# nayuki/DEFLATE-library-Java

Measured on AMD Instinct MI355X. Metric: input MiB/s (compress+decompress), higher is better.
Workload: dtype u8

## Files before the change

deflate-library-java_amd/csrc/hip/inflate_kernels.hip:

```cpp
#pragma once
#include "ndfl_common.hpp"
#include "../../../include/ndfl.h"
#include <vector>
#include <algorithm>
#include <unordered_map>
#include <chrono>
#include <string.h>
#include <stdio.h>
#include <stdlib.h>

namespace inf {

constexpr uint32_t SEG_BYTES = 65536;
constexpr uint32_t SEG_CAP = 256;
constexpr uint64_t NONE = ~0ull;

enum : uint32_t { ST_BOUNDARY = 0, ST_FINAL = 1, ST_ERROR = 2 };
constexpr int NEED_INPUT = 64;
enum : int { R_UEOS = 1, R_RESERVED_BLOCK_TYPE, R_LEN_MISMATCH, R_UNDER_FULL, R_OVER_FULL, R_NO_PREV,
             R_CL_OVER_FULL, R_EOB_ZERO, R_RESERVED_LEN, R_RESERVED_DIST, R_EMPTY_DIST, R_COPY_BEFORE,
             R_RESERVED_LEN_HI = 20, R_RESERVED_DIST_HI = 21,
             R_INTERNAL = 100 };

constexpr int CLO[19] = {16, 17, 18, 0, 8, 7, 9, 6, 10, 5, 11, 4, 12, 3, 13, 2, 14, 1, 15};
// ... 422 lines not shown
    __device__ __forceinline__ uint32_t pick8(uint32_t i) const {
        const uint32_t a = pick(cur, i), b = pick(nxt, i);
        return (i & 4) ? b : a;
    }
    __device__ __forceinline__ void load(const In& in, uint64_t g) {
        qw = g;
        cur = in.ld4(g);
        nxt = in.ld4(g + 1);
    }
    __device__ __forceinline__ uint64_t bits64(uint32_t o) const {
        const uint32_t i = o >> 5, sh = o & 31;
        const uint64_t x = (uint64_t)pick8(i) | ((uint64_t)pick8(i + 1) << 32);
        return sh ? (x >> sh) | ((uint64_t)pick8(i + 2) << (64 - sh)) : x;
    }
    __device__ __forceinline__ void fill() {
        if (bn <= 32 && fi < 8) { bb |= (uint64_t)pick8(fi) << bn; bn += 32; fi++; }
    }
    __device__ __forceinline__ void seek(uint64_t p) {
        pos = p;
        const uint32_t o = (uint32_t)(p - qw * 128);
        fi = o >> 5;
        bb = (uint64_t)(pick8(fi) >> (o & 31));
        bn = 32 - (o & 31);
        fi++;
        fill();
    }
    __device__ __forceinline__ bool starved() const { return bn <= 32 && fi >= 8; }
    __device__ __forceinline__ void reload(const In& in) {
        const uint64_t wn = qw * 4 + fi;
        load(in, wn >> 2);
        fi = (uint32_t)wn & 3u;
    }
    __device__ __forceinline__ uint32_t peek(uint32_t n) const { return (uint32_t)bb & ((1u << n) - 1u); }
    __device__ __forceinline__ void skip(uint32_t n) { bb >>= n; bn -= n; pos += n; }
};
}

extern "C" __global__ void __launch_bounds__(256) __attribute__((amdgpu_waves_per_eu(NDFL_STRICT_WPE)))
ndfl_inflate_strict_kernel(const uint32_t* w, uint64_t nwords, uint64_t nbits, const uint64_t* qlist,
                           const uint32_t* qcount, uint32_t qcap, uint32_t* seg_cnt, uint64_t* seg_list,
                           uint32_t* ticket, unsigned long long* sst) {
    using namespace inf;
    __shared__ uint4 tabs[256 * 8];
    uint8_t* tab = (uint8_t*)&tabs[threadIdx.x * 8];
    const uint32_t n = min(*qcount, qcap);
    In in{w, nwords, nbits};
    const uint32_t lane = threadIdx.x & 63u;
    uint32_t next = 0, end = 0;
    bool drained = false;
    const uint64_t below = (1ull << lane) - 1ull;
    auto record = [&](uint64_t p) {
        const uint32_t seg = (uint32_t)(p / ((uint64_t)SEG_BYTES * 8));
        const uint32_t idx = atomicAdd(&seg_cnt[seg], 1u);
        if (idx < SEG_CAP) seg_list[(uint64_t)seg * SEG_CAP + idx] = p;
    };
    bool active = false;
    uint64_t p = 0;
    SRd rd;
    rd.bb = 0; rd.pos = 0; rd.qw = 0; rd.bn = 0; rd.fi = 8;
    uint32_t i = 0, total = 0, numLit = 0, numDist = 0, litK = 0, distK = 0, nz = 0, eob = 0;
    int runVal = -1;
    uint64_t n_iter = 0, n_refill = 0, n_steps = 0;
    for (;;) {
        const uint64_t idle = __ballot(!active);
        const uint32_t nidle = (uint32_t)__popcll(idle);
        n_iter++;
        if (next >= end && !drained && nidle >= NDFL_STRICT_REFILL) {
            uint32_t t = 0;
            if (lane == 0) t = atomicAdd(ticket, STRICT_SLICE);
            t = __shfl(t, 0);
            if (t >= n) drained = true;
            else { next = t; end = min(n, t + STRICT_SLICE); }
        }
        if (next < end && nidle >= NDFL_STRICT_REFILL) {
            n_refill++;
            if (!active) {
                const uint32_t k = next + (uint32_t)__popcll(idle & below);
                if (k < end) {
                    const uint64_t e = qlist[k];
                    p = e & ~(1ull << 63);
                    if (!(e >> 63)) {
                        if (strict_stored(in, p)) record(p);
                    } else {
                        rd.load(in, p >> 7);
                        const uint32_t o = (uint32_t)p & 127u;
                        const uint32_t h = (uint32_t)rd.bits64(o + 3);
                        const uint32_t hlit = h & 31u, hdist = (h >> 5) & 31u, hclen = (h >> 10) & 15u;
                        numLit = hlit + 257; numDist = hdist + 1; total = numLit + numDist;
                        const uint32_t numCl = hclen + 4;
                        const uint64_t F = rd.bits64(o + 17) & ((1ull << (3 * numCl)) - 1ull);
                        rd.seek(p + 17 + 3 * numCl);
                        uint64_t wp = 0;
                        uint32_t kraft = 0;
#pragma unroll
                        for (int sy = 0; sy < 19; sy++) {
                            const uint32_t l = (uint32_t)(F >> (3 * CLO_INV[sy])) & 7u;
                            wp += l ? ((uint64_t)(128u >> l) << (8 * l)) : 0ull;
                            kraft += l ? (128u >> l) : 0u;
                        }
                        const bool complete = kraft == 128u;
                        uint64_t off = (wp * 0x0101010101010101ull) << 8;
#pragma unroll 1
                        for (int sy = 0; sy < 19; sy++) {
                            const uint32_t l = (uint32_t)(F >> (3 * CLO_INV[sy])) & 7u;
                            if (l && complete) {
                                const uint32_t sh = 8 * l, run = 128u >> l;
                                const uint32_t pos = (uint32_t)(off >> sh) & 255u;
                                off += (uint64_t)run << sh;
                                const uint32_t v = ((uint32_t)sy | (l << 5)) * 0x01010101u;
                                if (run >= 16) {
                                    for (uint32_t r = 0; r < run; r += 16) *(uint4*)(tab + pos + r) = make_uint4(v, v, v, v);
                                } else if (run == 8) {
                                    *(uint2*)(tab + pos) = make_uint2(v, v);
                                } else if (run == 4) {
                                    *(uint32_t*)(tab + pos) = v;
                                } else if (run == 2) {
                                    *(uint16_t*)(tab + pos) = (uint16_t)v;
                                } else {
                                    tab[pos] = (uint8_t)v;
                                }
                            }
                        }
                        i = 0; runVal = -1; litK = 0; distK = 0; nz = 0; eob = 0;
                        active = complete;
                    }
                }
            }
            next = min(end, next + nidle);
            continue;
        }
        if (!__any(active)) {
            if (next >= end && drained) break;
            continue;
        }
        const bool more = next < end || !drained;
        for (uint32_t ni = nidle;;) {
        n_steps += 64 - ni;
        if (__any(active && rd.starved())) {
            if (active && rd.fi >= 4) rd.reload(in);
        }
        if (active) {
            rd.fill();
            const uint32_t b = (uint32_t)rd.bb;
            const uint32_t te = tab[__builtin_bitreverse32(b) >> 25];
            const uint32_t sym = te & 31u, cl = te >> 5;
            const bool s16 = sym == 16, s17 = sym == 17, s18 = sym == 18;
            const uint32_t nx = s16 ? 2u : s17 ? 3u : s18 ? 7u : 0u;
            const uint32_t ex = (b >> cl) & ((1u << nx) - 1u);
            const uint32_t run = sym < 16 ? 1u : ex + (s18 ? 11u : 3u);
            const bool bad = s16 && runVal < 0;
            runVal = sym < 16 ? (int)sym : s16 ? runVal : 0;
            rd.skip(cl + nx);
            const uint32_t en = i + run;
            const uint32_t v = (uint32_t)runVal;
            const uint32_t wt = v ? (32768u >> v) : 0u;
            litK += (min(en, numLit) - min(i, numLit)) * wt;
            const uint32_t da = max(i, numLit) - numLit, db = max(en, numLit) - numLit, cd = db - da;
            distK += cd * wt;
            nz += v ? cd : 0u;
            eob = (i <= 256 && 256 < en) ? v : eob;
            i = en;
            const bool go = !(bad || en > total) && litK <= 32768u && distK <= 32768u;
            active = go && i < total;
            if (go && i >= total) {
                bool ok;
                if (eob == 0 || litK != 32768u || rd.pos > in.nbits) ok = false;
                else if (numDist == 1 && distK == 0) ok = true;
                else if (nz == 1 && distK == 16384u) ok = true;
                else ok = distK == 32768u;
                if (ok) record(p);
            }
        }
        const uint64_t am = __ballot(active);
        ni = 64u - (uint32_t)__popcll(am);
        if (!am || (more && ni >= NDFL_STRICT_REFILL)) break;
        n_iter++;
        }
    }
    if (sst && lane == 0) {
        atomicAdd(&sst[0], (unsigned long long)n_iter);
        atomicAdd(&sst[1], (unsigned long long)n_refill);
        atomicAdd(&sst[2], (unsigned long long)n_steps);
        atomicAdd(&sst[3], 1ull);
    }
}
extern "C" __global__ void __launch_bounds__(256)
ndfl_inflate_compact_kernel(const uint32_t* seg_cnt, const uint64_t* seg_list, const uint64_t* seg_off,
                            uint32_t nseg, uint64_t* out) {
    using namespace inf;
    __shared__ uint64_t sv[4][SEG_CAP];
    const uint32_t wid = threadIdx.x >> 6, lane = threadIdx.x & 63u;
    const uint32_t seg = blockIdx.x * 4 + wid;
    if (seg >= nseg) return;
    const uint32_t c = min(seg_cnt[seg], SEG_CAP);
    const uint64_t* src = seg_list + (uint64_t)seg * SEG_CAP;
    uint64_t* o = out + seg_off[seg];
    static_assert(SEG_CAP == 256, "four candidates per lane");
    uint64_t v[4];
#pragma unroll
    for (int q = 0; q < 4; q++) {
        const uint32_t i = lane + 64u * q;
        v[q] = i < c ? src[i] : ~0ull;
        if (i < c) sv[wid][i] = v[q];
    }
    __builtin_amdgcn_fence(__ATOMIC_RELEASE, "wavefront");
    __builtin_amdgcn_wave_barrier();
    __builtin_amdgcn_fence(__ATOMIC_ACQUIRE, "wavefront");
    uint32_t r[4] = {0, 0, 0, 0};
    for (uint32_t j = 0; j < c; j++) {
        const uint64_t u = sv[wid][j];
#pragma unroll
        for (int q = 0; q < 4; q++) r[q] += u < v[q] ? 1u : 0u;
    }
#pragma unroll
    for (int q = 0; q < 4; q++)
        if (lane + 64u * q < c) o[r[q]] = v[q];
}

struct ChainRes {
    uint64_t end_bit;
    uint64_t out_count;
    uint32_t status;
    uint32_t reason;
    uint32_t next;
    uint32_t pad;
    uint64_t bnd_bit;
    uint64_t bnd_cnt;
};

struct EmitChain {
    uint64_t start_bit;
    uint64_t end_bit;
    uint64_t out_off;
    uint64_t out_count;
    uint64_t slot;
};

enum : uint32_t { LI_NCAND = 0, LI_NCH, LI_TOTAL, LI_FLAGS, LI_STOP, LI_CODE, LI_OUTLEN, LI_CONSUMED, LI_NCAND_ALL,
                  LI_LO, LI_NREP, LI_NFLAT, LI_WORDS = 16 };
enum : uint64_t { LF_REPAIR = 1, LF_RANGE = 2, LF_CAPACITY = 4 };
constexpr uint32_t NOLINK = 0xFFFFFFFFu;

extern "C" __global__ void __launch_bounds__(SCAN_T)
ndfl_inflate_segsum_kernel(const uint32_t* cnt, uint32_t nseg, uint64_t* part) {
    using namespace inf;
    scan_tile_sum([&](uint32_t i) { return (uint64_t)min(cnt[i], SEG_CAP); }, nseg, part);
}
extern "C" __global__ void __launch_bounds__(SCAN_T)
ndfl_inflate_segscan_kernel(const uint32_t* cnt, uint32_t nseg, uint64_t* segoff, uint64_t* info, const uint64_t* part) {
    using namespace inf;
    scan_tile_apply([&](uint32_t i) { return (uint64_t)min(cnt[i], SEG_CAP); },
                    [&](uint32_t i, uint64_t v) { segoff[i] = v; }, nseg, part, 1, info + LI_NCAND_ALL);
}

extern "C" __global__ void __launch_bounds__(256)
ndfl_inflate_cand_slice_kernel(const uint64_t* sorted, uint64_t* info, uint64_t start_bit, uint64_t end_bit,
                               uint64_t* cands) {
    __shared__ uint64_t s_lo, s_hi;
    const uint64_t na = info[LI_NCAND_ALL];
    if (threadIdx.x == 0) {
        uint64_t lo = 1, hi = na;
        while (lo < hi) { const uint64_t m = (lo + hi) >> 1; if (sorted[m] <= start_bit) lo = m + 1; else hi = m; }
        uint64_t lo2 = lo, hi2 = na;
        while (lo2 < hi2) { const uint64_t m = (lo2 + hi2) >> 1; if (sorted[m] < end_bit) lo2 = m + 1; else hi2 = m; }
        s_lo = lo; s_hi = lo2;
        if (blockIdx.x == 0) { info[LI_NCAND] = 1 + (lo2 - lo); info[LI_LO] = lo; cands[0] = start_bit; }
    }
    __syncthreads();
    const uint64_t lo = s_lo, n = s_hi - s_lo;
    for (uint64_t k = (uint64_t)blockIdx.x * 256 + threadIdx.x; k < n; k += (uint64_t)gridDim.x * 256)
        cands[1 + k] = sorted[lo + k];
}

__device__ __forceinline__ uint64_t stored_key(const inf::In& in, uint64_t p) {
    const uint32_t h = (uint32_t)in.win64(p) & 7u;
    if ((h >> 1) != 0 || p + 3 > in.nbits) return ~0ull;
    return (((p + 3 + 7) & ~7ull) << 1) | (h & 1u);
}

extern "C" __global__ void __launch_bounds__(256)
ndfl_inflate_alias_mark_kernel(const uint64_t* cands, uint64_t* info, const uint32_t* w, uint64_t nwords, uint64_t nbits,
                               uint32_t* rep) {
    const inf::In in{w, nwords, nbits};
    const uint32_t n = (uint32_t)min<uint64_t>(info[LI_NCAND], 0xFFFFFFFFull);
    for (uint32_t k0 = blockIdx.x * 256; k0 < n; k0 += gridDim.x * 256) {
        const uint32_t k = k0 + threadIdx.x;
        bool own = false;
        if (k < n) {
            const uint64_t p = cands[k], key = stored_key(in, p);
            uint32_t r = k;
            if (key != ~0ull)
                for (uint32_t j = k; j > 0 && cands[j - 1] + 10 >= p; j--)
                    if (stored_key(in, cands[j - 1]) == key) r = j - 1;
            rep[k] = r;
            own = r == k;
        }
        const uint32_t c = (uint32_t)__popcll(__ballot(own));
        if ((threadIdx.x & 63) == 0 && c) atomicAdd((unsigned long long*)&info[LI_NREP], (unsigned long long)c);
    }
}

constexpr uint32_t OB_NB = 24;
constexpr uint32_t OB_WORDS = 2 * OB_NB;
constexpr size_t CTK_BYTES = 512;

template <class Bk>
__device__ __forceinline__ void border_count(Bk bk, uint32_t n, uint32_t* ob) {
    __shared__ uint32_t h[OB_NB];
    const uint32_t t = threadIdx.x;
    if (t < OB_NB) h[t] = 0;
    __syncthreads();
    const uint32_t i0 = blockIdx.x * SCAN_TILE + t * SCAN_PER;
    if (i0 < n) {
        uint32_t b[SCAN_PER];
#pragma unroll
        for (uint32_t k = 0; k < SCAN_PER; k++) b[k] = bk(min(i0 + k, n - 1));
#pragma unroll
        for (uint32_t k = 0; k < SCAN_PER; k++) if (i0 + k < n && b[k] < OB_NB) atomicAdd(&h[b[k]], 1u);
    }
    __syncthreads();
    if (t < OB_NB && h[t]) atomicAdd(&ob[t], h[t]);
}
template <class Bk>
__device__ __forceinline__ void border_place(Bk bk, uint32_t n, uint32_t* ob, uint32_t* order, uint32_t* ntot) {
    __shared__ uint32_t h[OB_NB], base[OB_NB];
    const uint32_t t = threadIdx.x;
    if (t < OB_NB) h[t] = 0;
    __syncthreads();
    const uint32_t i0 = blockIdx.x * SCAN_TILE + t * SCAN_PER;
    uint32_t b[SCAN_PER];
#pragma unroll
    for (uint32_t k = 0; k < SCAN_PER; k++) b[k] = OB_NB;
    if (i0 < n) {
#pragma unroll
        for (uint32_t k = 0; k < SCAN_PER; k++) b[k] = bk(min(i0 + k, n - 1));
#pragma unroll
        for (uint32_t k = 0; k < SCAN_PER; k++) {
            if (i0 + k >= n) b[k] = OB_NB;
            if (b[k] < OB_NB) atomicAdd(&h[b[k]], 1u);
        }
    }
    __syncthreads();
    if (t < OB_NB) {
        uint32_t p = 0;
        for (uint32_t q = 0; q < t; q++) p += ob[q];
        base[t] = p + (h[t] ? atomicAdd(&ob[OB_NB + t], h[t]) : 0u);
        h[t] = 0;
    }
    __syncthreads();
#pragma unroll
    for (uint32_t k = 0; k < SCAN_PER; k++)
        if (b[k] < OB_NB) order[base[b[k]] + atomicAdd(&h[b[k]], 1u)] = i0 + k;
    if (ntot && blockIdx.x == 0 && t == 0) {
        uint32_t p = 0;
        for (uint32_t q = 0; q < OB_NB; q++) p += ob[q];
        *ntot = p;
    }
}

struct OrderBucket {
    const uint64_t* cands; uint32_t n; uint64_t end_bit; const uint32_t* rep; const uint32_t* flat;
    __device__ __forceinline__ uint32_t operator()(uint32_t k) const {
        const uint64_t c0 = cands[k], c1 = cands[min(k + 1, n - 1)];
        const uint32_t r = rep ? rep[k] : k;
        const uint64_t nx = k + 1 < n ? c1 : end_bit;
        const uint64_t len = nx > c0 ? nx - c0 : 0;
        if (flat && flat[k]) return OB_NB;
        return r == k ? OB_NB - 1 - (uint32_t)min<uint64_t>(OB_NB - 1, len >> 15) : OB_NB;
    }
};
extern "C" __global__ void __launch_bounds__(SCAN_T)
ndfl_inflate_order_count_kernel(const uint64_t* cands, uint32_t n, uint64_t end_bit, const uint32_t* rep, uint32_t* ob,
                                const uint32_t* flat) {
    border_count(OrderBucket{cands, n, end_bit, rep, flat}, n, ob);
}
extern "C" __global__ void __launch_bounds__(SCAN_T)
ndfl_inflate_order_kernel(const uint64_t* cands, uint32_t n, uint64_t end_bit, uint32_t* order, const uint32_t* rep,
                          uint32_t* nord, uint32_t* ob, const uint32_t* flat) {
    border_place(OrderBucket{cands, n, end_bit, rep, flat}, n, ob, order, nord);
}

struct EmitBucket {
    const EmitChain* chains;
    __device__ __forceinline__ uint32_t operator()(uint32_t k) const {
        const EmitChain& e = chains[k];
        const uint64_t key = ((e.end_bit - e.start_bit) >> 15) + (e.out_count >> 14);
        return OB_NB - 1 - (uint32_t)min<uint64_t>(OB_NB - 1, key);
    }
};
extern "C" __global__ void __launch_bounds__(SCAN_T)
ndfl_inflate_emit_order_count_kernel(const EmitChain* chains, const uint64_t* info, uint32_t* ob) {
    if (info[LI_FLAGS]) return;
    border_count(EmitBucket{chains}, (uint32_t)info[LI_NCH], ob);
}
extern "C" __global__ void __launch_bounds__(SCAN_T)
ndfl_inflate_emit_order_kernel(const EmitChain* chains, const uint64_t* info, uint32_t* order, uint32_t* ob) {
    if (info[LI_FLAGS]) return;
    border_place(EmitBucket{chains}, (uint32_t)info[LI_NCH], ob, order, (uint32_t*)nullptr);
}

extern "C" __global__ void __launch_bounds__(256)
ndfl_inflate_link_init_kernel(const ChainRes* res, uint32_t n, const uint64_t* cands, uint64_t end_bit, uint32_t* J0,
                              uint64_t* S, uint32_t* D) {
    using namespace inf;
    for (uint32_t k = blockIdx.x * 256 + threadIdx.x; k < n; k += gridDim.x * 256) {
        const ChainRes r = res[k];
        const bool lk = r.status == ST_BOUNDARY && r.end_bit < end_bit && r.next < n && cands[r.next] == r.end_bit;
        J0[k] = lk ? r.next : NOLINK;
        S[k] = r.out_count;
        D[k] = lk ? 1u : 0u;
    }
}
extern "C" __global__ void __launch_bounds__(256)
ndfl_inflate_link_jump_kernel(const uint32_t* J, uint32_t* J2, const uint64_t* S, uint64_t* S2, const uint32_t* D,
                              uint32_t* D2, uint32_t n) {
    for (uint32_t k = blockIdx.x * 256 + threadIdx.x; k < n; k += gridDim.x * 256) {
        const uint32_t j = J[k];
        if (j != NOLINK) { J2[k] = J[j]; S2[k] = S[k] + S[j]; D2[k] = D[k] + D[j]; }
        else { J2[k] = NOLINK; S2[k] = S[k]; D2[k] = D[k]; }
    }
}
extern "C" __global__ void __launch_bounds__(256)
ndfl_inflate_link_path_kernel(const uint32_t* Jall, uint32_t nlev, const uint64_t* S, const uint32_t* D,
                              const ChainRes* res, const uint64_t* cands, uint32_t n, uint64_t dict_len, uint64_t end_bit,
                              uint64_t out_cap, EmitChain* chains, uint64_t* info) {
    using namespace inf;
    const uint32_t len = D[0] + 1;
    for (uint32_t t = blockIdx.x * 256 + threadIdx.x; t < len; t += gridDim.x * 256) {
        uint32_t node = 0;
        for (uint32_t r = 0; r < nlev; r++)
            if ((t >> r) & 1u) node = Jall[(uint64_t)r * n + node];
        const ChainRes c = res[node];
        EmitChain e;
        e.start_bit = cands[node];
        e.end_bit = c.end_bit;
        e.out_off = dict_len + S[0] - S[node];
        e.out_count = c.out_count;
        e.slot = node;
        chains[t] = e;
        if (t + 1 == len) {
            uint64_t flags = 0, stop = 0;
            if (c.status == ST_FINAL) stop = c.end_bit;
            else if (c.status == ST_BOUNDARY) {
                if (c.end_bit == end_bit) stop = end_bit;
                else if (c.end_bit > end_bit) flags |= LF_RANGE;
                else flags |= LF_REPAIR;
            }
            if (S[0] > out_cap) flags |= LF_CAPACITY;
            info[LI_NCH] = len; info[LI_TOTAL] = S[0]; info[LI_FLAGS] = flags; info[LI_STOP] = stop;
        }
    }
}
extern "C" __global__ void __launch_bounds__(SCAN_T)
ndfl_inflate_first_error_kernel(const ChainRes* er, const uint64_t* info, uint32_t* first) {
    using namespace inf;
    const uint32_t nch = (uint32_t)info[LI_NCH];
    const uint32_t i0 = blockIdx.x * SCAN_TILE + threadIdx.x * SCAN_PER;
    if (i0 >= nch) return;
    uint32_t st[SCAN_PER];
#pragma unroll
    for (uint32_t k = 0; k < SCAN_PER; k++) st[k] = er[min(i0 + k, nch - 1)].status;
#pragma unroll
    for (uint32_t k = 0; k < SCAN_PER; k++)
        if (i0 + k < nch && st[k] == ST_ERROR) { atomicMin(first, i0 + k); break; }
}
extern "C" __global__ void __launch_bounds__(64)
ndfl_inflate_summary_kernel(const ChainRes* er, const EmitChain* chains, uint64_t* info, uint64_t dict_len,
                            uint32_t partial, const uint32_t* firstp) {
    using namespace inf;
    if (threadIdx.x != 0) return;
    const uint32_t first = *firstp;
    if (first == NOLINK) {
        info[LI_CODE] = 0; info[LI_OUTLEN] = info[LI_TOTAL]; info[LI_CONSUMED] = info[LI_STOP];
        return;
    }
    const ChainRes r = er[first];
    if (partial && r.reason == R_UEOS) {
        info[LI_CODE] = NEED_INPUT;
        info[LI_OUTLEN] = chains[first].out_off - dict_len + r.bnd_cnt;
        info[LI_CONSUMED] = r.bnd_bit;
    } else {
        info[LI_CODE] = r.reason;
        info[LI_OUTLEN] = chains[first].out_off - dict_len + r.out_count;
        info[LI_CONSUMED] = r.end_bit;
    }
}

#include "inflate_records.hpp"
static_assert((CT_ORDER + 2 * OB_WORDS + 1) * 4 <= CTK_BYTES, "ticket buffer layout");
#include "inflate_wave.hpp"
#include "inflate_wg.hpp"

extern "C" __global__ void __launch_bounds__(256)
ndfl_inflate_alias_copy_kernel(const uint32_t* rep, uint32_t n, ChainRes* res, SegPool pool) {
    for (uint32_t k = blockIdx.x * 256 + threadIdx.x; k < n; k += gridDim.x * 256) {
        const uint32_t r = rep[k];
        if (r == k) continue;
        res[k] = res[r];
        if (k < pool.nslot) pool.head[k] = r < pool.nslot ? pool.head[r] : NOREC;
    }
}


struct InflateScratch {
    void* d_in = nullptr; size_t d_in_cap = 0;
    void* d_cand = nullptr; size_t d_cand_cap = 0;
    void* d_starts = nullptr; size_t d_starts_cap = 0;
    void* d_stops = nullptr; size_t d_stops_cap = 0;
    void* d_res = nullptr; size_t d_res_cap = 0;
    void* d_cands = nullptr; size_t d_cands_cap = 0;
    void* d_stats = nullptr;
    void* d_q = nullptr; size_t d_q_cap = 0;
    void* d_seg = nullptr; size_t d_seg_cap = 0;
    SegPool pool{};
    void* d_chains = nullptr; size_t d_chains_cap = 0;
    void* d_off = nullptr; size_t d_off_cap = 0;
    void* d_ref = nullptr; size_t d_ref_cap = 0;
    void* d_pend = nullptr; size_t d_pend_cap = 0;
    void* d_rl = nullptr; size_t d_rl_cap = 0;
    void* d_ticket = nullptr;
    void* d_slow = nullptr; size_t d_slow_cap = 0;
    void* d_rep = nullptr; size_t d_rep_cap = 0;
    void* d_ph = nullptr;
    void* d_hrec = nullptr;
    size_t d_hrec_cap = 0;
    void* d_cticket = nullptr;
    void* d_out = nullptr; size_t d_out_cap = 0;
    Knobs knobs;
    uint32_t q_cap = 0, q_min = 0;
    bool q_full = false;
    double last_ms_find = 0, last_ms_count = 0, last_ms_emit = 0, last_ms_wall = 0;
    hipEvent_t ev[6] = {nullptr, nullptr, nullptr, nullptr, nullptr, nullptr};
    uint64_t repairs = 0, chains = 0, candidates = 0, resolved_groups = 0, flat_chains = 0;
    uint64_t pending_after_dev = 0;
    void* h_cnt = nullptr;
    void* d_info = nullptr;
    void* h_info = nullptr;
    void* d_link = nullptr; size_t d_link_cap = 0;
    bool count_first = false;
    bool pending = false;
    uint8_t* p_out = nullptr;
    uint64_t p_nbytes = 0, p_dict_len = 0;
    void release() {
        void** ps[] = {&d_in, &d_cand, &d_starts, &d_stops, &d_res, &d_cands, &d_stats, &d_q, &d_seg, &d_chains, &d_off,
                       &d_ref, &d_pend, &d_rl, &d_ticket, &d_ph, &d_cticket, &d_out, &d_hrec, &d_slow, &d_rep};
        for (void** p : ps) { if (*p) hipFree(*p); *p = nullptr; }
        for (auto& e : ev) { if (e) hipEventDestroy(e); e = nullptr; }
        if (h_cnt) hipHostFree(h_cnt);
        h_cnt = nullptr;
        if (h_info) hipHostFree(h_info);
        h_info = nullptr;
        if (d_info) hipFree(d_info);
        d_info = nullptr;
        if (d_link) hipFree(d_link);
        d_link = nullptr; d_link_cap = 0;
        d_in_cap = d_cand_cap = d_starts_cap = d_stops_cap = d_res_cap = d_cands_cap = d_seg_cap = d_q_cap = d_chains_cap = 0;
        d_off_cap = d_ref_cap = d_pend_cap = d_rl_cap = d_out_cap = d_hrec_cap = 0;
        pending = false;
    }
};

template <typename K>
static uint32_t wave_grid(K kernel, uint32_t cap, const char* env = nullptr) {
    int dev = 0, ncu = 0, per = 0;
    if (hipGetDevice(&dev) != hipSuccess || hipDeviceGetAttribute(&ncu, hipDeviceAttributeMultiprocessorCount, dev) != hipSuccess ||
        hipOccupancyMaxActiveBlocksPerMultiprocessor(&per, kernel, 64, 0) != hipSuccess || ncu <= 0 || per <= 0)
        return cap;
    if (env && getenv(env)) per = std::max(1, atoi(getenv(env)));
    return std::min<uint32_t>(cap, (uint32_t)(ncu * per));
}

static uint32_t count_w(const Knobs& k) {
    const uint32_t v = k.count_w ? k.count_w : (uint32_t)NDFL_COUNT_W_DEFAULT;
    return (v == 2 || v == 4 || v == 8) ? v : 1u;
}
template <typename K>
static uint32_t wg_grid(K kernel, uint32_t threads, uint32_t cap) {
    int dev = 0, ncu = 0, per = 0;
    if (hipGetDevice(&dev) != hipSuccess || hipDeviceGetAttribute(&ncu, hipDeviceAttributeMultiprocessorCount, dev) != hipSuccess ||
        hipOccupancyMaxActiveBlocksPerMultiprocessor(&per, kernel, (int)threads, 0) != hipSuccess || ncu <= 0 || per <= 0)
        return cap;
    return std::min<uint32_t>(cap, (uint32_t)(ncu * per));
}
template <typename... A>
static void launch_count(hipStream_t s, uint32_t W, uint32_t nchains, A... args) {
    if (W == 1) {
        static const uint32_t g1 = wave_grid(ndfl_inflate_count_wave_kernel, inf::COUNT_WAVES, "NDFL_COUNT_WPC");
        hipLaunchKernelGGL(ndfl_inflate_count_wave_kernel, dim3(std::min(nchains, g1)), dim3(64), 0, s, args...);
    } else if (W == 2) {
        static const uint32_t g = wg_grid(ndfl_inflate_count_wg_kernel<2>, 128, inf::COUNT_WAVES / 2);
        hipLaunchKernelGGL(ndfl_inflate_count_wg_kernel<2>, dim3(std::min(nchains, g)), dim3(128), 0, s, args...);
    } else if (W == 4) {
        static const uint32_t g = wg_grid(ndfl_inflate_count_wg_kernel<4>, 256, inf::COUNT_WAVES / 4);
        hipLaunchKernelGGL(ndfl_inflate_count_wg_kernel<4>, dim3(std::min(nchains, g)), dim3(256), 0, s, args...);
    } else {
        static const uint32_t g = wg_grid(ndfl_inflate_count_wg_kernel<8>, 512, inf::COUNT_WAVES / 8);
        hipLaunchKernelGGL(ndfl_inflate_count_wg_kernel<8>, dim3(std::min(nchains, g)), dim3(512), 0, s, args...);
    }
}

static hipError_t inf_ensure(void** p, size_t* cap, size_t n) {
    if (n <= *cap && *p) return hipSuccess;
    if (*p) { hipFree(*p); *p = nullptr; *cap = 0; }
    size_t want = n < 4096 ? 4096 : n;
    hipError_t e = hipMalloc(p, want);
    if (e == hipSuccess) *cap = want;
    return e;
}


static bool inf_debug() { static const bool d = getenv("NDFL_DEBUG") != nullptr; return d; }
#define INF_CHK(x) do { hipError_t _e = (x); if (_e != hipSuccess) {                                             \
        if (inf_debug()) fprintf(stderr, "[ndfl] HIP error %d (%s) at inflate_kernels.hip:%d\n", (int)_e,     \
                                 hipGetErrorString(_e), __LINE__);                                              \
        return -4; } } while (0)
#define INF_RC(x) do { const int _r = (x); if (_r) return _r; } while (0)

static int resolve_rounds(InflateScratch& S, hipStream_t s, uint8_t* d_out, uint64_t nbytes, uint64_t* groups) {
    using namespace inf;
    *groups = 0;
    const uint64_t npw = (nbytes + 31) / 32;
    if (npw == 0) return 0;
    if (npw > 0xFFFFFFFFull) return -2;
    INF_CHK(inf_ensure(&S.d_rl, &S.d_rl_cap, npw * 12 + 64));
    uint32_t* cnt = (uint32_t*)S.d_rl;
    uint32_t* lst[2] = {(uint32_t*)((char*)S.d_rl + 64), (uint32_t*)((char*)S.d_rl + 64) + npw};
    uint32_t* nb = lst[1] + npw;
    uint32_t* pend = (uint32_t*)S.d_pend;
    uint32_t* ref = (uint32_t*)S.d_ref;
    INF_CHK(hipMemsetAsync(cnt, 0, 8, s));
    hipLaunchKernelGGL(ndfl_inflate_pending_list_kernel, dim3((uint32_t)((npw + 4095) / 4096)), dim3(256), 0, s,
                       (const uint32_t*)pend, (uint64_t)0, npw, lst[0], cnt);
    INF_CHK(hipGetLastError());
    if (!S.h_cnt) INF_CHK(hipHostMalloc(&S.h_cnt, 64, 0));
    uint32_t* h = (uint32_t*)S.h_cnt;
    int cur = 0;
    uint32_t n = 0;
    for (int round = 0;; round++) {
        const bool rstats = S.knobs.stats;
        if ((round & 3) == 0 || rstats) {
            INF_CHK(hipMemcpyAsync(h, cnt + cur, 4, hipMemcpyDeviceToHost, s));
            if (rstats) INF_CHK(hipMemcpyAsync(h + 1, cnt + 2 + cur, 4, hipMemcpyDeviceToHost, s));
            INF_CHK(hipStreamSynchronize(s));
            n = *h;
            if (rstats) fprintf(stderr, "[ndfl] resolve round %d: %u pending groups, %u bytes\n", round, n, h[1]);
            if (round == 0) *groups = n;
            if (n == 0) return 0;
            if (round >= 96) return R_INTERNAL;
        }
        INF_CHK(hipMemsetAsync(cnt + (cur ^ 1), 0, 4, s));
        if (rstats) INF_CHK(hipMemsetAsync(cnt + 2 + (cur ^ 1), 0, 4, s));
        const uint32_t gb = (uint32_t)std::min<uint64_t>(4096, ((uint64_t)n * 32 + 255) / 256);
        hipLaunchKernelGGL(ndfl_inflate_resolve_kernel, dim3(gb), dim3(256), 0, s,
                           (const uint32_t*)lst[cur], (const uint32_t*)(cnt + cur), (const uint32_t*)pend, ref, d_out, nb);
        INF_CHK(hipGetLastError());
        hipLaunchKernelGGL(ndfl_inflate_resolve_apply_kernel, dim3((uint32_t)std::min<uint64_t>(1024, (n + 255) / 256)),
                           dim3(256), 0, s, (const uint32_t*)lst[cur], (const uint32_t*)(cnt + cur), pend,
                           (const uint32_t*)nb, lst[cur ^ 1], cnt + (cur ^ 1), rstats ? cnt + 2 + (cur ^ 1) : (uint32_t*)nullptr);
        INF_CHK(hipGetLastError());
        cur ^= 1;
    }
}

static int print_count_stats(InflateScratch& S, bool phase_clock_note) {
    uint32_t st[64] = {0};
    INF_CHK(hipMemcpy(st, S.d_stats, 256, hipMemcpyDeviceToHost));
    const unsigned long long* ss = (const unsigned long long*)(st + SW_STRICT64);
    fprintf(stderr, "[ndfl] strict stage: %llu waves, %llu loop trips (%llu refills), %llu lane-symbol steps\n",
            ss[3], ss[0], ss[1], ss[2]);
    const uint64_t* t64 = (const uint64_t*)(st + SW_CLOCK64);
    fprintf(stderr, "[ndfl] count wave-time (ms x waves, 100 MHz clock%s): header %.1f spec %.1f "
            "verify %.1f phases %.1f serial %.1f record %.1f build %.1f phase-mapped %.1f\n",
            phase_clock_note ? "; -DNDFL_PHASE_CLOCK builds" : "", t64[0] * 1e-5,
            t64[1] * 1e-5, t64[2] * 1e-5, t64[3] * 1e-5, t64[4] * 1e-5, t64[5] * 1e-5, t64[6] * 1e-5, t64[7] * 1e-5);
    const double span = (double)(t64[9] - ~t64[10]);
    fprintf(stderr, "[ndfl] count waves %llu: busy %.1f ms x waves, span %.3f ms, occupancy %.3f, longest chain %.3f ms\n",
            (unsigned long long)t64[11], t64[8] * 1e-5, span * 1e-5, t64[11] ? t64[8] / (span * t64[11]) : 0.0,
            t64[12] * 1e-5);
    return 0;
}

static int setup_pool(InflateScratch& S, hipStream_t s, uint64_t nstarts, uint64_t nbits) {
    using namespace inf;
    const uint64_t nslot = nstarts + std::max<uint64_t>(4096, nstarts / 2);
    const uint64_t nrec = std::min<uint64_t>(0xFFFFFFF0ull, 2 * nstarts + nbits / (wv::MAX_SPAN / 2) + 65536);
    const uint64_t nbt = std::min<uint64_t>(nrec, S.knobs.no_bt ? 0 : (1u << 18));
    const uint64_t seg_bytes = nrec * (64 * 8 + 64 * 4 + sizeof(SegMeta)) + nslot * 4 + 64 + nbt * BT_BYTES;
    INF_CHK(inf_ensure(&S.d_seg, &S.d_seg_cap, seg_bytes));
    SegPool pool;
    pool.start = (uint64_t*)S.d_seg;
    pool.cnt = (uint32_t*)(pool.start + nrec * 64);
    pool.meta = (SegMeta*)(pool.cnt + nrec * 64);
    pool.head = (uint32_t*)(pool.meta + nrec);
    pool.ctr = (uint32_t*)S.d_stats + SW_REC_CTR;
    pool.bctr = (uint32_t*)S.d_stats + SW_TREC_CTR;
    pool.nbt = (uint32_t)nbt;
    pool.bt = (TabRec*)(((uintptr_t)(pool.head + nslot) + 63) & ~(uintptr_t)63);
    pool.nrec = (uint32_t)nrec;
    pool.nslot = nslot;
    S.pool = pool;
    INF_CHK(hipMemsetAsync(pool.head, 0xFF, nslot * 4, s));
    return 0;
}

static int resolve_rounds_dev(InflateScratch& S, hipStream_t s, uint8_t* d_out, uint64_t nbytes, int rounds,
                              uint32_t** left, uint64_t* first_count_dst) {
    using namespace inf;
    const uint64_t npw = (nbytes + 31) / 32;
    *left = nullptr;
    if (npw == 0) return 0;
    if (npw > 0xFFFFFFFFull) return -2;
    INF_CHK(inf_ensure(&S.d_rl, &S.d_rl_cap, npw * 12 + 64));
    uint32_t* cnt = (uint32_t*)S.d_rl;
    uint32_t* lst[2] = {(uint32_t*)((char*)S.d_rl + 64), (uint32_t*)((char*)S.d_rl + 64) + npw};
    uint32_t* nb = lst[1] + npw;
    uint32_t* pend = (uint32_t*)S.d_pend;
    uint32_t* ref = (uint32_t*)S.d_ref;
    INF_CHK(hipMemsetAsync(cnt, 0, 8, s));
    hipLaunchKernelGGL(ndfl_inflate_pending_list_kernel, dim3((uint32_t)((npw + 4095) / 4096)), dim3(256), 0, s,
                       (const uint32_t*)pend, (uint64_t)0, npw, lst[0], cnt);
    INF_CHK(hipGetLastError());
    if (first_count_dst) INF_CHK(hipMemcpyAsync(first_count_dst, cnt, 4, hipMemcpyDeviceToDevice, s));
    int cur = 0;
    for (int round = 0; round < rounds; round++) {
        INF_CHK(hipMemsetAsync(cnt + (cur ^ 1), 0, 4, s));
        hipLaunchKernelGGL(ndfl_inflate_resolve_kernel, dim3(4096), dim3(256), 0, s, (const uint32_t*)lst[cur],
                           (const uint32_t*)(cnt + cur), (const uint32_t*)pend, ref, d_out, nb);
        INF_CHK(hipGetLastError());
        hipLaunchKernelGGL(ndfl_inflate_resolve_apply_kernel, dim3(1024), dim3(256), 0, s, (const uint32_t*)lst[cur],
                           (const uint32_t*)(cnt + cur), pend, (const uint32_t*)nb, lst[cur ^ 1], cnt + (cur ^ 1),
                           (uint32_t*)nullptr);
        INF_CHK(hipGetLastError());
        cur ^= 1;
    }
    *left = cnt + cur;
    return 0;
}

constexpr int LINK_FALLBACK = 1000;
constexpr int FIND_OVERFLOW = 1001;
constexpr uint32_t LI_QCOUNT = 14;

static int inflate_devlink(InflateScratch& S, hipStream_t s, const uint32_t* d_w, uint64_t nwords, uint64_t nbits,
                           uint32_t nseg, const uint32_t* d_cnt, const uint64_t* d_list, uint64_t start_bit,
                           uint64_t end_bit, uint8_t* out, uint64_t dict_len, uint64_t out_cap, uint64_t* out_len,
                           uint64_t* consumed_bits, uint32_t flags, bool deferred, bool partial, double* last_ms) {
    using namespace inf;
    if (!S.d_info) INF_CHK(hipMalloc(&S.d_info, LI_WORDS * 8));
    if (!S.h_info) INF_CHK(hipHostMalloc(&S.h_info, LI_WORDS * 8, 0));
    uint64_t* info = (uint64_t*)S.d_info;
    volatile uint64_t* hinfo = (volatile uint64_t*)S.h_info;
    INF_CHK(hipMemsetAsync(info, 0, LI_WORDS * 8, s));
    const uint64_t cap_all = (uint64_t)nseg * SEG_CAP + 1;
    const uint32_t ntile = (nseg + SCAN_TILE - 1) / SCAN_TILE;
    INF_CHK(inf_ensure(&S.d_starts, &S.d_starts_cap, (cap_all + nseg + 2 + ntile) * 8));
    uint64_t* d_sorted = (uint64_t*)S.d_starts;
    uint64_t* d_segoff = d_sorted + cap_all;
    uint64_t* d_part = d_segoff + nseg + 2;
    hipLaunchKernelGGL(ndfl_inflate_segsum_kernel, dim3(ntile), dim3(SCAN_T), 0, s, d_cnt, nseg, d_part);
    INF_CHK(hipGetLastError());
    hipLaunchKernelGGL(ndfl_inflate_segscan_kernel, dim3(ntile), dim3(SCAN_T), 0, s, d_cnt, nseg, d_segoff, info,
                       (const uint64_t*)d_part);
    INF_CHK(hipGetLastError());
    hipLaunchKernelGGL(ndfl_inflate_compact_kernel, dim3((nseg + 3) / 4), dim3(256), 0, s, d_cnt, d_list,
                       (const uint64_t*)d_segoff, nseg, d_sorted);
    INF_CHK(hipGetLastError());
    INF_CHK(inf_ensure(&S.d_cands, &S.d_cands_cap, (cap_all + 1) * 8ull));
    hipLaunchKernelGGL(ndfl_inflate_cand_slice_kernel, dim3((uint32_t)std::min<uint64_t>(4096, (cap_all + 255) / 256)),
                       dim3(256), 0, s, (const uint64_t*)d_sorted, info, start_bit, end_bit, (uint64_t*)S.d_cands);
    INF_CHK(hipGetLastError());
    const bool alias_on = !S.knobs.no_alias;
    uint32_t* d_rep = nullptr;
    if (alias_on) {
        INF_CHK(inf_ensure(&S.d_rep, &S.d_rep_cap, (size_t)cap_all * 4 + 64));
        d_rep = (uint32_t*)S.d_rep;
        hipLaunchKernelGGL(ndfl_inflate_alias_mark_kernel, dim3((uint32_t)std::min<uint64_t>(1024, (cap_all + 255) / 256)),
                           dim3(256), 0, s, (const uint64_t*)S.d_cands, info, d_w, nwords, nbits, d_rep);
        INF_CHK(hipGetLastError());
    }
    INF_CHK(hipMemcpyAsync((void*)hinfo, info, (LI_NREP + 1) * 8, hipMemcpyDeviceToHost, s));
    hinfo[LI_QCOUNT] = 0;
    INF_CHK(hipMemcpyAsync((void*)(hinfo + LI_QCOUNT), (const uint32_t*)S.d_stats + SW_QCOUNT, 4, hipMemcpyDeviceToHost, s));
    INF_CHK(hipStreamSynchronize(s));
    if ((uint32_t)hinfo[LI_QCOUNT] > S.q_cap && !S.q_full) { S.q_min = (uint32_t)hinfo[LI_QCOUNT] + 65536; return FIND_OVERFLOW; }
    const uint64_t n = hinfo[LI_NCAND];
    const uint64_t nrep = alias_on ? hinfo[LI_NREP] : n;
    static const uint32_t count_waves = wave_grid(ndfl_inflate_count_wave_kernel, COUNT_WAVES, "NDFL_COUNT_WPC");
    const uint32_t W = S.knobs.count_w ? count_w(S.knobs) : (nrep < 2ull * count_waves && nbits >= (1ull << 24)) ? 4u : 1u;
    if (S.knobs.stats) fprintf(stderr, "[ndfl] count pass: %llu candidates, %llu counted, width %u\n",
                                      (unsigned long long)n, (unsigned long long)nrep, W);
    if (n == 0 || n > (1ull << 24)) return LINK_FALLBACK;
    const uint32_t ncand = (uint32_t)n;
    int rc = setup_pool(S, s, n, nbits);
    if (rc) return rc;
    INF_CHK(inf_ensure(&S.d_stops, &S.d_stops_cap, n * 12));
    INF_CHK(inf_ensure(&S.d_res, &S.d_res_cap, n * sizeof(ChainRes)));
    uint32_t* d_order = (uint32_t*)((char*)S.d_stops + n * 8);
    if (!S.d_cticket) INF_CHK(hipMalloc(&S.d_cticket, CTK_BYTES));
    INF_CHK(hipMemsetAsync(S.d_cticket, 0, CTK_BYTES, s));
    uint32_t* d_nord = (uint32_t*)S.d_cticket + CT_NORD;
    uint32_t* d_nflat = (uint32_t*)S.d_cticket + CT_NFLAT;
    uint32_t* d_ob = (uint32_t*)S.d_cticket + CT_ORDER;
    const uint32_t otiles = (ncand + SCAN_TILE - 1) / SCAN_TILE;
    if (!S.d_ph) INF_CHK(hipMalloc(&S.d_ph, (size_t)std::max(COUNT_WAVES, EMIT_WAVES) * sizeof(wv::PhArr)));
    const bool stats_on = S.knobs.stats;
    const uint64_t limit = std::min(end_bit, nbits);
    INF_CHK(hipEventRecord(S.ev[2], s));
    const bool hrec_on = !S.knobs.no_hdrrec;
    const bool flat_on = hrec_on && W == 1 && S.knobs.flat && nrep >= S.knobs.flat_min;
    uint32_t* d_flist = nullptr;
    uint32_t* d_fflag = nullptr;
    if (hrec_on) {
        INF_CHK(inf_ensure(&S.d_hrec, &S.d_hrec_cap, (size_t)ncand * (sizeof(wv::HdrRec) + 8) + 64));
        d_flist = (uint32_t*)((char*)S.d_hrec + (size_t)ncand * sizeof(wv::HdrRec));
        d_fflag = d_flist + ncand;
        hipLaunchKernelGGL(ndfl_inflate_hdr_kernel, dim3((ncand + 63) / 64), dim3(64), 0, s, d_w, nwords, nbits,
                           (const uint64_t*)S.d_cands, ncand, (wv::HdrRec*)S.d_hrec, flat_on ? d_flist : nullptr,
                           d_nflat, flat_on ? d_fflag : nullptr);
        INF_CHK(hipGetLastError());
    }
    hipLaunchKernelGGL(ndfl_inflate_order_count_kernel, dim3(otiles), dim3(SCAN_T), 0, s, (const uint64_t*)S.d_cands,
                       ncand, end_bit, (const uint32_t*)d_rep, d_ob, flat_on ? (const uint32_t*)d_fflag : nullptr);
    INF_CHK(hipGetLastError());
    hipLaunchKernelGGL(ndfl_inflate_order_kernel, dim3(otiles), dim3(SCAN_T), 0, s, (const uint64_t*)S.d_cands, ncand,
                       end_bit, d_order, (const uint32_t*)d_rep, (alias_on || flat_on) ? d_nord : (uint32_t*)nullptr, d_ob,
                       flat_on ? (const uint32_t*)d_fflag : nullptr);
    INF_CHK(hipGetLastError());
    if (flat_on) INF_CHK(hipMemcpyAsync(info + LI_NFLAT, d_nflat, 4, hipMemcpyDeviceToDevice, s));
    launch_count(s, W, ncand,
                       d_w, nwords, nbits, (const uint64_t*)S.d_cands, (const uint64_t*)nullptr, ncand,
                       (const uint64_t*)S.d_cands, ncand, limit, (ChainRes*)S.d_res,
                       stats_on ? (uint32_t*)S.d_stats : nullptr, (uint64_t)0, S.pool, (uint32_t*)S.d_cticket,
                       (wv::PhArr*)S.d_ph, (const uint32_t*)d_order, end_bit,
                       hrec_on ? (const wv::HdrRec*)S.d_hrec : nullptr,
                       (alias_on || flat_on) ? (const uint32_t*)d_nord : nullptr, flat_on ? (const uint32_t*)d_flist : nullptr,
                       flat_on ? (const uint32_t*)d_nflat : nullptr);
    INF_CHK(hipGetLastError());
    if (alias_on) {
        hipLaunchKernelGGL(ndfl_inflate_alias_copy_kernel, dim3(std::min<uint32_t>(1024, (ncand + 255) / 256)), dim3(256), 0, s,
                           (const uint32_t*)d_rep, ncand, (ChainRes*)S.d_res, S.pool);
        INF_CHK(hipGetLastError());
    }
    INF_CHK(hipEventRecord(S.ev[3], s));
    if (stats_on) {
        std::vector<ChainRes> cr(ncand);
        INF_CHK(hipMemcpyAsync(cr.data(), S.d_res, ncand * sizeof(ChainRes), hipMemcpyDeviceToHost, s));
        INF_CHK(hipStreamSynchronize(s));
        uint64_t cnt[3] = {0, 0, 0}, tsum[3] = {0, 0, 0}, tmax[3] = {0, 0, 0}, blk[3] = {0, 0, 0};
        for (uint32_t k = 0; k < ncand; k++) {
            const uint32_t st = std::min<uint32_t>(cr[k].status, 2u), t = cr[k].pad >> 16;
            cnt[st]++; tsum[st] += t; tmax[st] = std::max<uint64_t>(tmax[st], t); blk[st] += cr[k].pad & 0xFFFFu;
        }
        if (flat_on) {
            uint32_t fw[CT_ORDER] = {0};
            INF_CHK(hipMemcpy(fw, S.d_cticket, sizeof(fw), hipMemcpyDeviceToHost));
            const uint32_t* why = fw + CT_FLAT_WHY;
            fprintf(stderr, "[ndfl] count flat groups sent back: (unused) %u, full-table tokens %u, "
                    "error %u, chain goes on %u, table %u\n", why[1], why[2], why[3], why[4], why[5]);
            const uint32_t nfl = fw[CT_NFLAT];
            const unsigned long long gt = (unsigned long long)fw[CT_FLAT_TIME64] | ((unsigned long long)fw[CT_FLAT_TIME64 + 1] << 32);
            fprintf(stderr, "[ndfl] count flat groups: %u chains in %u groups, %u sent back to the wave decode, "
                    "group wave time %.3f ms mean\n", nfl, (nfl + 63) / 64, fw[CT_FLAT_REDO], nfl ? gt * 1e-5 / ((nfl + 63) / 64) : 0.0);
#ifdef NDFL_FLAT_PROF
            unsigned long long fpv[4] = {0, 0, 0, 0}, z[4] = {0, 0, 0, 0};
            INF_CHK(hipMemcpyFromSymbol(fpv, HIP_SYMBOL(wv::g_flat_prof), 32));
            INF_CHK(hipMemcpyToSymbol(HIP_SYMBOL(wv::g_flat_prof), z, 32));
            fprintf(stderr, "[ndfl] flat decode loops (lane 0, clock64): %llu cycles, %llu at %llu phase points\n", fpv[0], fpv[1], fpv[2]);
#endif
        }
        const char* nm[3] = {"boundary", "final", "error"};
        for (int k = 0; k < 3; k++)
            fprintf(stderr, "[ndfl] count chains %s: %llu, wave time %.2f ms (max %.3f ms), blocks %llu\n", nm[k],
                    (unsigned long long)cnt[k], tsum[k] * 1e-2, tmax[k] * 1e-2, (unsigned long long)blk[k]);
        std::vector<uint64_t> cb(ncand);
        INF_CHK(hipMemcpy(cb.data(), S.d_cands, ncand * 8, hipMemcpyDeviceToHost));
        uint64_t bn[OB_NB] = {}, bt[OB_NB] = {}, bm[OB_NB] = {};
        uint32_t bk[OB_NB] = {};
        std::vector<uint32_t> top;
        for (uint32_t k = 0; k < ncand; k++) {
            const uint64_t nx = k + 1 < ncand ? cb[k + 1] : end_bit, len = nx > cb[k] ? nx - cb[k] : 0;
            const uint32_t b = (uint32_t)std::min<uint64_t>(OB_NB - 1, len >> 15), t = cr[k].pad >> 16;
            bn[b]++; bt[b] += t;
            if (t >= bm[b]) { bm[b] = t; bk[b] = k; }
            top.push_back(k);
        }
        for (uint32_t b = 0; b < OB_NB; b++)
            if (bn[b]) fprintf(stderr, "[ndfl] count bits %2u x 32Ki: %6llu chains, mean %.3f ms, max %.3f ms "
                               "(chain %u at bit %llu: blocks %u, status %u, out %llu)\n", b,
                               (unsigned long long)bn[b], bt[b] * 1e-2 / bn[b], bm[b] * 1e-2, bk[b],
                               (unsigned long long)cb[bk[b]], cr[bk[b]].pad & 0xFFFFu, cr[bk[b]].status,
                               (unsigned long long)cr[bk[b]].out_count);
        const size_t nt = std::min<size_t>(8, top.size());
        std::partial_sort(top.begin(), top.begin() + nt, top.end(),
                          [&](uint32_t a, uint32_t b) { return (cr[a].pad >> 16) > (cr[b].pad >> 16); });
        for (size_t i = 0; i < nt; i++) {
            const uint32_t k = top[i];
            const uint64_t nx = k + 1 < ncand ? cb[k + 1] : end_bit;
            fprintf(stderr, "[ndfl] count longest: chain %u at bit %llu, %llu bits, %.3f ms, blocks %u, status %u, out %llu\n",
                    k, (unsigned long long)cb[k], (unsigned long long)(nx - cb[k]), (cr[k].pad >> 16) * 1e-2,
                    cr[k].pad & 0xFFFFu, cr[k].status, (unsigned long long)cr[k].out_count);
        }
    }
    uint32_t nlev = 1;
    while ((1ull << nlev) < n) nlev++;
    const size_t link_bytes = (size_t)(nlev + 1) * n * 4 + 2 * n * 8 + 2 * n * 4 + 64;
    INF_CHK(inf_ensure(&S.d_link, &S.d_link_cap, link_bytes));
    uint32_t* J = (uint32_t*)S.d_link;
    uint64_t* Ssum[2] = {(uint64_t*)(((uintptr_t)(J + (size_t)(nlev + 1) * n) + 7) & ~(uintptr_t)7), nullptr};
    Ssum[1] = Ssum[0] + n;
    uint32_t* Dd[2] = {(uint32_t*)(Ssum[1] + n), nullptr};
    Dd[1] = Dd[0] + n;
    const uint32_t lg = (uint32_t)std::min<uint64_t>(4096, (n + 255) / 256);
    hipLaunchKernelGGL(ndfl_inflate_link_init_kernel, dim3(lg), dim3(256), 0, s, (const ChainRes*)S.d_res, ncand,
                       (const uint64_t*)S.d_cands, end_bit, J, Ssum[0], Dd[0]);
    INF_CHK(hipGetLastError());
    int cur = 0;
    for (uint32_t r = 0; r < nlev; r++) {
        hipLaunchKernelGGL(ndfl_inflate_link_jump_kernel, dim3(lg), dim3(256), 0, s, (const uint32_t*)(J + (size_t)r * n),
                           J + (size_t)(r + 1) * n, (const uint64_t*)Ssum[cur], Ssum[cur ^ 1], (const uint32_t*)Dd[cur],
                           Dd[cur ^ 1], ncand);
        INF_CHK(hipGetLastError());
        cur ^= 1;
    }
    INF_CHK(inf_ensure(&S.d_chains, &S.d_chains_cap, n * sizeof(EmitChain)));
    hipLaunchKernelGGL(ndfl_inflate_link_path_kernel, dim3(lg), dim3(256), 0, s, (const uint32_t*)J, nlev,
                       (const uint64_t*)Ssum[cur], (const uint32_t*)Dd[cur], (const ChainRes*)S.d_res,
                       (const uint64_t*)S.d_cands, ncand, dict_len, end_bit, out_cap, (EmitChain*)S.d_chains, info);
    INF_CHK(hipGetLastError());
    {
        uint32_t* d_eob = (uint32_t*)S.d_cticket + CT_ORDER + OB_WORDS;
        const uint32_t etiles = (ncand + SCAN_TILE - 1) / SCAN_TILE;
        hipLaunchKernelGGL(ndfl_inflate_emit_order_count_kernel, dim3(etiles), dim3(SCAN_T), 0, s,
                           (const EmitChain*)S.d_chains, (const uint64_t*)info, d_eob);
        INF_CHK(hipGetLastError());
        hipLaunchKernelGGL(ndfl_inflate_emit_order_kernel, dim3(etiles), dim3(SCAN_T), 0, s, (const EmitChain*)S.d_chains,
                           (const uint64_t*)info, d_order, d_eob);
        INF_CHK(hipGetLastError());
    }
    uint8_t* d_out;
    const bool direct = (flags & 2u) != 0;
    const uint64_t obytes = dict_len + std::min<uint64_t>(out_cap, 129 * nbits + 65536);
    if (obytes > (40ull << 30)) return LINK_FALLBACK;
    if (direct) d_out = out;
    else {
        INF_CHK(inf_ensure(&S.d_out, &S.d_out_cap, obytes + 64));
        d_out = (uint8_t*)S.d_out;
        if (dict_len) INF_CHK(hipMemcpyAsync(d_out, out, dict_len, hipMemcpyHostToDevice, s));
    }
    const uint64_t nbytes = obytes;
    if ((nbytes + 31) / 32 > 0xFFFFFFFFull) return LINK_FALLBACK;
    const uint64_t npw = (nbytes + 31) / 32;
    INF_CHK(inf_ensure(&S.d_ref, &S.d_ref_cap, nbytes * 4 + 64));
    INF_CHK(inf_ensure(&S.d_pend, &S.d_pend_cap, npw * 4 + 64));
    INF_CHK(hipMemsetAsync(S.d_pend, 0, npw * 4 + 64, s));
    if (!S.d_ticket) INF_CHK(hipMalloc(&S.d_ticket, 64));
    INF_CHK(hipMemsetAsync(S.d_ticket, 0, 64, s));
    if (S.knobs.test_segflip && S.pool.cnt) {
        uint32_t c0 = 0;
        INF_CHK(hipMemcpyAsync(&c0, S.pool.cnt, 4, hipMemcpyDeviceToHost, s));
        INF_CHK(hipStreamSynchronize(s));
        c0++;
        INF_CHK(hipMemcpyAsync(S.pool.cnt, &c0, 4, hipMemcpyHostToDevice, s));
        INF_CHK(hipStreamSynchronize(s));
    }
    INF_CHK(hipEventRecord(S.ev[4], s));
    static const uint32_t emit_grid = wave_grid(ndfl_inflate_emit_wave_kernel, EMIT_WAVES, "NDFL_EMIT_WPC");
    if (S.knobs.emit_fast) {
        INF_CHK(inf_ensure(&S.d_slow, &S.d_slow_cap, (size_t)ncand * 4 + 64));
        uint32_t* tk = (uint32_t*)S.d_ticket;
        static const uint32_t fast_grid = wave_grid(ndfl_inflate_emit_fast_kernel, EMIT_WAVES, "NDFL_EMITF_WPC");
        hipLaunchKernelGGL(ndfl_inflate_emit_fast_kernel, dim3(std::min<uint32_t>(ncand, fast_grid)), dim3(64), 0, s, d_w,
                           nwords, nbits, (const EmitChain*)S.d_chains, tk, d_out, (ChainRes*)S.d_res,
                           (uint32_t*)S.d_ref, (uint32_t*)S.d_pend, S.pool, (const uint64_t*)info, (const uint32_t*)d_order,
                           (uint32_t*)S.d_slow, tk + 8);
        INF_CHK(hipGetLastError());
        hipLaunchKernelGGL(ndfl_inflate_emit_wave_kernel, dim3(std::min<uint32_t>(ncand, emit_grid)), dim3(64), 0, s, d_w,
                           nwords, nbits, (const EmitChain*)S.d_chains, ncand, tk + 4, d_out,
                           (ChainRes*)S.d_res, (const uint64_t*)S.d_cands, ncand, (uint32_t*)S.d_ref, (uint32_t*)S.d_pend,
                           S.pool, (wv::PhArr*)S.d_ph, stats_on ? (uint32_t*)S.d_stats : nullptr, (const uint64_t*)info,
                           (const uint32_t*)S.d_slow, (const uint32_t*)(tk + 8));
        INF_CHK(hipGetLastError());
        if (stats_on) {
            uint32_t nsl = 0;
            INF_CHK(hipMemcpyAsync(&nsl, tk + 8, 4, hipMemcpyDeviceToHost, s));
            INF_CHK(hipStreamSynchronize(s));
            fprintf(stderr, "[ndfl] fast emit pass left %u chains to the full emit pass\n", nsl);
        }
    } else {
        hipLaunchKernelGGL(ndfl_inflate_emit_wave_kernel, dim3(std::min<uint32_t>(ncand, emit_grid)), dim3(64), 0, s, d_w,
                           nwords, nbits, (const EmitChain*)S.d_chains, ncand, (uint32_t*)S.d_ticket, d_out,
                           (ChainRes*)S.d_res, (const uint64_t*)S.d_cands, ncand, (uint32_t*)S.d_ref, (uint32_t*)S.d_pend,
                           S.pool, (wv::PhArr*)S.d_ph, stats_on ? (uint32_t*)S.d_stats : nullptr, (const uint64_t*)info,
                           (const uint32_t*)d_order, (const uint32_t*)nullptr);
        INF_CHK(hipGetLastError());
    }
    INF_CHK(hipEventRecord(S.ev[5], s));
    {
        uint32_t* d_first = (uint32_t*)S.d_cticket + CT_ORDER + 2 * OB_WORDS;
        INF_CHK(hipMemsetAsync(d_first, 0xFF, 4, s));
        hipLaunchKernelGGL(ndfl_inflate_first_error_kernel, dim3((ncand + SCAN_TILE - 1) / SCAN_TILE), dim3(SCAN_T), 0, s,
                           (const ChainRes*)S.d_res, (const uint64_t*)info, d_first);
        INF_CHK(hipGetLastError());
        hipLaunchKernelGGL(ndfl_inflate_summary_kernel, dim3(1), dim3(64), 0, s, (const ChainRes*)S.d_res,
                           (const EmitChain*)S.d_chains, info, dict_len, partial ? 1u : 0u, (const uint32_t*)d_first);
        INF_CHK(hipGetLastError());
    }
    uint32_t* left = nullptr;
    if (!deferred) {
        rc = resolve_rounds_dev(S, s, d_out, nbytes, 6, &left, stats_on ? info + LI_WORDS - 3 : (uint64_t*)nullptr);
        if (rc) return rc;
        if (left) INF_CHK(hipMemcpyAsync(info + LI_WORDS - 1, left, 4, hipMemcpyDeviceToDevice, s));
    }
    INF_CHK(hipMemcpyAsync((void*)hinfo, info, LI_WORDS * 8, hipMemcpyDeviceToHost, s));
    INF_CHK(hipStreamSynchronize(s));
    if (stats_on) {
        uint32_t st[3] = {0, 0, 0};
        INF_CHK(hipMemcpy(st, S.d_stats, sizeof(st), hipMemcpyDeviceToHost));
        fprintf(stderr, "[ndfl] device link: chains %llu of %u candidates; count pass: slow-verify lanes %u fixups %u "
                "rounds %u\n", (unsigned long long)hinfo[LI_NCH], ncand, st[SW_NSLOW], st[SW_NFIX], st[SW_NROUND]);
        fprintf(stderr, "[ndfl] emit: %u pending 32-byte groups before the resolve rounds, %u after six\n",
                (uint32_t)(hinfo[LI_WORDS - 3] & 0xFFFFFFFFu), (uint32_t)(hinfo[LI_WORDS - 1] & 0xFFFFFFFFu));
        rc = print_count_stats(S, true);
        if (rc) return rc;
    }
    const uint64_t lflags = hinfo[LI_FLAGS];
    if (lflags & LF_REPAIR) return LINK_FALLBACK;
    if (lflags & LF_RANGE) return -1;
    S.chains = hinfo[LI_NCH];
    S.candidates = ncand;
    S.flat_chains = hinfo[LI_NFLAT];
    S.repairs = 0;
    if (lflags & LF_CAPACITY) { *out_len = hinfo[LI_TOTAL]; return -3; }
    const uint32_t pending_left = (uint32_t)(hinfo[LI_WORDS - 1] & 0xFFFFFFFFu);
    S.pending_after_dev = deferred ? 0 : pending_left;
    if (!deferred && pending_left) {
        uint64_t groups = 0;
        rc = resolve_rounds(S, s, d_out, nbytes, &groups);
        if (rc) return rc;
    }
    {
        float a = 0, b = 0, c = 0;
        hipEventElapsedTime(&a, S.ev[0], S.ev[1]);
        hipEventElapsedTime(&b, S.ev[2], S.ev[3]);
        hipEventElapsedTime(&c, S.ev[4], S.ev[5]);
        S.last_ms_find = a; S.last_ms_count = b; S.last_ms_emit = c;
    }
    if (deferred) { S.pending = true; S.p_out = d_out; S.p_nbytes = dict_len + hinfo[LI_TOTAL]; S.p_dict_len = dict_len; }
    INF_CHK(hipEventRecord(S.ev[5], s));
    INF_CHK(hipStreamSynchronize(s));
    float w = 0;
    hipEventElapsedTime(&w, S.ev[0], S.ev[5]);
    S.last_ms_wall = w;
    *last_ms = w;
    const int code = (int)hinfo[LI_CODE];
    const uint64_t produced = hinfo[LI_OUTLEN];
    if (!direct && produced) INF_CHK(hipMemcpy(out + dict_len, d_out + dict_len, produced, hipMemcpyDeviceToHost));
    *out_len = produced;
    *consumed_bits = hinfo[LI_CONSUMED];
    return code;
}

static int stage_input(InflateScratch& S, hipStream_t s, const uint8_t* in, uint64_t in_len, uint32_t flags,
                       const uint32_t** d_w) {
    using namespace inf;
    const uint64_t nwords = (in_len + 3) / 4;
    const bool in_place = in_len && (flags & 1u) && (flags & 8u) && ((uintptr_t)in & 15u) == 0;
    *d_w = (const uint32_t*)in;
    if (!in_place) {
        INF_CHK(inf_ensure(&S.d_in, &S.d_in_cap, nwords * 4 + IN_PAD));
        if (in_len) INF_CHK(hipMemcpyAsync(S.d_in, in, in_len, (flags & 1u) ? hipMemcpyDeviceToDevice : hipMemcpyHostToDevice, s));
        INF_CHK(hipMemsetAsync((char*)S.d_in + in_len, 0, nwords * 4 + IN_PAD - in_len, s));
        *d_w = (const uint32_t*)S.d_in;
    }
    return 0;
}

static int find_headers(InflateScratch& S, hipStream_t s, const uint32_t* d_w, uint64_t nwords, uint64_t nbits,
                        uint64_t start_bit, uint64_t end_bit, uint32_t* d_cnt, uint64_t* d_list) {
    using namespace inf;
    const uint64_t scan_end = std::min(end_bit, nbits);
    const uint64_t w_lo = start_bit >> 5;
    const uint64_t nw32 = scan_end > w_lo * 32 ? (scan_end + 31) / 32 - w_lo : 0;
    constexpr uint64_t Q_BUDGET = (1ull << 30) / 8;
    const uint64_t qbase = std::min<uint64_t>(0x7FFFFFFFull, nbits / 256 + 65536);
    const uint64_t qtop = std::min<uint64_t>(0x7FFFFFFFull, std::max(qbase, Q_BUDGET));
    uint32_t qcap = (uint32_t)std::max(qbase, std::min<uint64_t>(S.q_min, qtop));
    S.q_full = qcap >= qtop;
    if (inf_ensure(&S.d_q, &S.d_q_cap, (uint64_t)qcap * 8 + 64) != hipSuccess) {
        (void)hipGetLastError();
        qcap = (uint32_t)qbase;
        S.q_full = true;
        S.q_min = 0;
        INF_CHK(inf_ensure(&S.d_q, &S.d_q_cap, (uint64_t)qcap * 8 + 64));
    }
    S.q_cap = qcap;
    uint32_t* d_qcount = (uint32_t*)S.d_stats + SW_QCOUNT;
    uint64_t* d_qlist = (uint64_t*)((char*)S.d_q + 64);
    static const uint32_t strict_grid = [] {
        int dev = 0, ncu = 0, per = 0;
        if (hipGetDevice(&dev) != hipSuccess ||
            hipDeviceGetAttribute(&ncu, hipDeviceAttributeMultiprocessorCount, dev) != hipSuccess ||
            hipOccupancyMaxActiveBlocksPerMultiprocessor(&per, ndfl_inflate_strict_kernel, 256, 0) != hipSuccess ||
            ncu <= 0 || per <= 0)
            return 1280u;
        return (uint32_t)(ncu * per);
    }();
    unsigned long long* sst = S.knobs.stats ? (unsigned long long*)((uint32_t*)S.d_stats + SW_STRICT64) : nullptr;
    if (nw32) {
        const uint32_t fgrid = (uint32_t)((nw32 + 256 * FIND_WPT - 1) / (256 * FIND_WPT));
        hipLaunchKernelGGL(ndfl_inflate_find_compact_kernel, dim3(fgrid), dim3(256), 0, s, d_w, nwords, nbits, d_qlist,
                           d_qcount, qcap, w_lo, scan_end);
        INF_CHK(hipGetLastError());
        hipLaunchKernelGGL(ndfl_inflate_strict_kernel, dim3(strict_grid), dim3(256), 0, s, d_w, nwords, nbits,
                           (const uint64_t*)d_qlist, (const uint32_t*)d_qcount, qcap, d_cnt, d_list,
                           (uint32_t*)S.d_stats + SW_STRICT_TICKET, sst);
        INF_CHK(hipGetLastError());
    }
    return 0;
}

static int inflate_headers(InflateScratch& S, hipStream_t s, const uint8_t* in, uint64_t in_len, uint32_t flags,
                           uint64_t* out, uint64_t cap, uint64_t* n_out, uint64_t* surv, uint64_t surv_cap,
                           uint64_t* stats) {
    using namespace inf;
    const uint64_t nbits = in_len * 8, nwords = (in_len + 3) / 4;
    const uint32_t* d_w = nullptr;
    INF_RC(stage_input(S, s, in, in_len, flags, &d_w));
    if (!S.d_stats) INF_CHK(hipMalloc(&S.d_stats, 512));
    const uint32_t nseg = (uint32_t)std::max<uint64_t>(1, (in_len + SEG_BYTES - 1) / SEG_BYTES);
    INF_CHK(inf_ensure(&S.d_cand, &S.d_cand_cap, (uint64_t)nseg * SEG_CAP * 8ull + (uint64_t)nseg * 4 + 64));
    uint64_t* d_list = (uint64_t*)S.d_cand;
    uint32_t* d_cnt = (uint32_t*)((char*)S.d_cand + (uint64_t)nseg * SEG_CAP * 8ull);
    std::vector<uint32_t> cnt(nseg);
    std::vector<uint64_t> lists((uint64_t)nseg * SEG_CAP);
    uint32_t qc = 0;
    for (int finds = 0; finds < 2; finds++) {
        INF_CHK(hipMemsetAsync(S.d_stats, 0, 512, s));
        INF_CHK(hipMemsetAsync(d_cnt, 0, (uint64_t)nseg * 4, s));
        INF_RC(find_headers(S, s, d_w, nwords, nbits, 0, NONE, d_cnt, d_list));
        INF_CHK(hipMemcpyAsync(&qc, (uint32_t*)S.d_stats + SW_QCOUNT, 4, hipMemcpyDeviceToHost, s));
        INF_CHK(hipStreamSynchronize(s));
        if (qc <= S.q_cap || S.q_full) break;
        S.q_min = qc + 65536;
    }
    INF_CHK(hipMemcpyAsync(cnt.data(), d_cnt, nseg * 4ull, hipMemcpyDeviceToHost, s));
    INF_CHK(hipMemcpyAsync(lists.data(), d_list, lists.size() * 8, hipMemcpyDeviceToHost, s));
    INF_CHK(hipStreamSynchronize(s));
    const uint32_t qcap = S.q_cap;
    std::vector<uint64_t> acc;
    uint64_t total = 0, over = 0;
    for (uint32_t k = 0; k < nseg; k++) {
        total += cnt[k];
        over += cnt[k] > SEG_CAP;
        for (uint32_t i = 0; i < std::min(cnt[k], SEG_CAP); i++) acc.push_back(lists[(uint64_t)k * SEG_CAP + i]);
    }
    std::sort(acc.begin(), acc.end());
    *n_out = acc.size();
    if (out) memcpy(out, acc.data(), std::min<uint64_t>(cap, acc.size()) * 8);
    if (surv && surv_cap) {
        const uint64_t ns = std::min<uint64_t>(std::min<uint64_t>(qc, qcap), surv_cap);
        if (ns) INF_CHK(hipMemcpy(surv, (const char*)S.d_q + 64, ns * 8, hipMemcpyDeviceToHost));
    }
    if (stats) { stats[0] = qc; stats[1] = total; stats[2] = over; stats[3] = qc > qcap ? qc - qcap : 0; }
    return 0;
}

static int inflate_run(InflateScratch& S, hipStream_t s, const uint8_t* in, uint64_t in_len, uint64_t start_bit,
                       uint64_t end_bit, uint8_t* out, uint64_t dict_len, uint64_t out_cap, uint64_t* out_len,
                       uint64_t* consumed_bits, uint32_t flags, bool deferred, double* last_ms, bool partial = false,
                       uint64_t* probe_sync = nullptr) {
    using namespace inf;
    *out_len = 0;
    *consumed_bits = 0;
    S.pending = false;
    if (!probe_sync) S.pending_after_dev = 0;
    const bool htime = S.knobs.host_times;
    auto hnow = []() { return std::chrono::duration<double, std::milli>(std::chrono::steady_clock::now().time_since_epoch()).count(); };
    double ht[8] = {hnow(), 0, 0, 0, 0, 0, 0, 0};
    const uint64_t nbits = in_len * 8;
    const uint64_t nwords = (in_len + 3) / 4;
    if (start_bit > nbits) return -1;
    const uint32_t* d_w = nullptr;
    INF_RC(stage_input(S, s, in, in_len, flags, &d_w));
    if (!S.d_stats) INF_CHK(hipMalloc(&S.d_stats, 512));
    if (!S.ev[0]) for (auto& e : S.ev) INF_CHK(hipEventCreate(&e));
    int finds = 0;
refind:
    INF_CHK(hipMemsetAsync(S.d_stats, 0, 512, s));
    const uint32_t nseg = (uint32_t)std::max<uint64_t>(1, (in_len + SEG_BYTES - 1) / SEG_BYTES);
    INF_CHK(inf_ensure(&S.d_cand, &S.d_cand_cap, (uint64_t)nseg * SEG_CAP * 8ull + (uint64_t)nseg * 4 + 64));
    uint64_t* d_list = (uint64_t*)S.d_cand;
    uint32_t* d_cnt = (uint32_t*)((char*)S.d_cand + (uint64_t)nseg * SEG_CAP * 8ull);
    INF_CHK(hipMemsetAsync(d_cnt, 0, (uint64_t)nseg * 4, s));
    INF_CHK(hipEventRecord(S.ev[0], s));
    INF_RC(find_headers(S, s, d_w, nwords, nbits, start_bit, end_bit, d_cnt, d_list));
    INF_CHK(hipEventRecord(S.ev[1], s));
    {
        const bool host_link = S.knobs.host_link;
        if (!probe_sync && !host_link) {
            const int rc = inflate_devlink(S, s, d_w, nwords, nbits, nseg, d_cnt, d_list, start_bit, end_bit, out,
                                           dict_len, out_cap, out_len, consumed_bits, flags, deferred, partial, last_ms);
            if (rc == FIND_OVERFLOW && finds++ == 0) goto refind;
            if (rc != LINK_FALLBACK && rc != FIND_OVERFLOW) return rc;
        }
    }
    std::vector<uint32_t> hcnt(nseg);
    uint32_t hqc = 0;
    INF_CHK(hipMemcpyAsync(hcnt.data(), d_cnt, nseg * 4ull, hipMemcpyDeviceToHost, s));
    INF_CHK(hipMemcpyAsync(&hqc, (const uint32_t*)S.d_stats + SW_QCOUNT, 4, hipMemcpyDeviceToHost, s));
    INF_CHK(hipStreamSynchronize(s));
    if (hqc > S.q_cap && !S.q_full && finds++ == 0) { S.q_min = hqc + 65536; goto refind; }
    std::vector<uint64_t> hoff(nseg + 1);
    hoff[0] = 1;
    for (uint32_t k = 0; k < nseg; k++) hoff[k + 1] = hoff[k] + std::min(hcnt[k], SEG_CAP);
    const uint64_t ncand_all = hoff[nseg];
    INF_CHK(inf_ensure(&S.d_starts, &S.d_starts_cap, (ncand_all + nseg + 2) * 8));
    uint64_t* d_sorted = (uint64_t*)S.d_starts;
    uint64_t* d_segoff = d_sorted + ncand_all;
    INF_CHK(hipMemcpyAsync(d_segoff, hoff.data(), nseg * 8ull, hipMemcpyHostToDevice, s));
    hipLaunchKernelGGL(ndfl_inflate_compact_kernel, dim3((nseg + 3) / 4), dim3(256), 0, s, (const uint32_t*)d_cnt,
                       (const uint64_t*)d_list, (const uint64_t*)d_segoff, nseg, d_sorted);
    INF_CHK(hipGetLastError());
    std::vector<uint64_t> starts(ncand_all);
    INF_CHK(hipMemcpyAsync(starts.data() + 1, d_sorted + 1, (ncand_all - 1) * 8, hipMemcpyDeviceToHost, s));
    INF_CHK(hipStreamSynchronize(s));
    starts[0] = start_bit;
    {
        size_t m = 1;
        for (size_t k = 1; k < starts.size(); k++)
            if (starts[k] > start_bit && starts[k] < end_bit) starts[m++] = starts[k];
        starts.resize(m);
    }
    const std::vector<uint64_t> sorted_cand(starts);
    const uint32_t ncand = (uint32_t)sorted_cand.size();
    INF_CHK(inf_ensure(&S.d_cands, &S.d_cands_cap, (ncand + 1) * 8ull));
    INF_CHK(hipMemcpyAsync(S.d_cands, sorted_cand.data(), ncand * 8ull, hipMemcpyHostToDevice, s));
    const uint64_t limit = std::min(end_bit, nbits);
    {
        const int prc = setup_pool(S, s, starts.size(), nbits);
        if (prc) return prc;
    }
    const SegPool pool = S.pool;

    const bool stats_on = S.knobs.stats;
    std::vector<ChainRes> res;
    auto run_count = [&](const std::vector<uint64_t>& st, std::vector<ChainRes>& r) -> int {
        const uint64_t slot_base = starts.size() - (&st == &starts ? st.size() : 0);
        const size_t n = st.size();
        std::vector<uint64_t> sp(n);
        for (size_t k = 0; k < n; k++) sp[k] = end_bit;
        std::vector<uint32_t> order(n);
        {
            constexpr int NB = 24;
            uint32_t bc[NB + 1] = {0};
            auto bucket = [&](size_t k) {
                const uint64_t nx = k + 1 < n ? st[k + 1] : end_bit;
                const uint64_t len = nx > st[k] ? nx - st[k] : 0;
                return NB - 1 - (int)std::min<uint64_t>(NB - 1, len >> 15);
            };
            const bool sorted_st = std::is_sorted(st.begin(), st.end());
            if (sorted_st) {
                for (size_t k = 0; k < n; k++) bc[bucket(k) + 1]++;
                for (int b = 0; b < NB; b++) bc[b + 1] += bc[b];
                for (size_t k = 0; k < n; k++) order[bc[bucket(k)]++] = (uint32_t)k;
            } else {
                for (size_t k = 0; k < n; k++) order[k] = (uint32_t)k;
            }
        }
        INF_CHK(inf_ensure(&S.d_starts, &S.d_starts_cap, n * 8));
        INF_CHK(inf_ensure(&S.d_stops, &S.d_stops_cap, n * 12));
        INF_CHK(inf_ensure(&S.d_res, &S.d_res_cap, n * sizeof(ChainRes)));
        INF_CHK(hipMemcpyAsync(S.d_starts, st.data(), n * 8, hipMemcpyHostToDevice, s));
        INF_CHK(hipMemcpyAsync(S.d_stops, sp.data(), n * 8, hipMemcpyHostToDevice, s));
        uint32_t* d_order = (uint32_t*)((char*)S.d_stops + n * 8);
        INF_CHK(hipMemcpyAsync(d_order, order.data(), n * 4, hipMemcpyHostToDevice, s));
        if (!S.d_ph) INF_CHK(hipMalloc(&S.d_ph, (size_t)std::max(COUNT_WAVES, EMIT_WAVES) * sizeof(wv::PhArr)));
        if (!S.d_cticket) INF_CHK(hipMalloc(&S.d_cticket, CTK_BYTES));
        INF_CHK(hipMemsetAsync(S.d_cticket, 0, 4, s));
        if (S.count_first) INF_CHK(hipEventRecord(S.ev[2], s));
        launch_count(s, count_w(S.knobs), (uint32_t)n,
                           d_w, nwords, nbits,
                           (const uint64_t*)S.d_starts, (const uint64_t*)S.d_stops, (uint32_t)n,
                           (const uint64_t*)S.d_cands, ncand, limit, (ChainRes*)S.d_res, stats_on ? (uint32_t*)S.d_stats : nullptr,
                           slot_base, pool, (uint32_t*)S.d_cticket, (wv::PhArr*)S.d_ph, (const uint32_t*)d_order,
                           end_bit, (const wv::HdrRec*)nullptr, (const uint32_t*)nullptr, (const uint32_t*)nullptr,
                           (const uint32_t*)nullptr);
        INF_CHK(hipGetLastError());
        if (S.count_first) { INF_CHK(hipEventRecord(S.ev[3], s)); S.count_first = false; }
        r.resize(n);
        INF_CHK(hipMemcpyAsync(r.data(), S.d_res, n * sizeof(ChainRes), hipMemcpyDeviceToHost, s));
        INF_CHK(hipStreamSynchronize(s));
        return 0;
    };
    ht[1] = hnow();
    S.repairs = 0;
    S.count_first = true;
    int rc = run_count(starts, res);
    if (rc) return rc;
    if (probe_sync) {
        *probe_sync = NONE;
        auto linked = [&](size_t k) {
            return res[k].status == ST_BOUNDARY && res[k].next < starts.size() && starts[res[k].next] == res[k].end_bit;
        };
        for (size_t k = 1; k < res.size(); k++) {
            if (!linked(k)) continue;
            const size_t j = res[k].next;
            if (j >= 1 && (linked(j) || res[j].status == ST_FINAL)) { *probe_sync = starts[j]; break; }
        }
        return 0;
    }
    if (S.knobs.stats && !probe_sync) {
        std::vector<size_t> idx(res.size());
        for (size_t k = 0; k < idx.size(); k++) idx[k] = k;
        const size_t top = std::min<size_t>(8, idx.size());
        std::partial_sort(idx.begin(), idx.begin() + top, idx.end(),
                          [&](size_t a, size_t b) { return (res[a].pad >> 16) > (res[b].pad >> 16); });
        for (size_t t = 0; t < top; t++) {
            const ChainRes& r = res[idx[t]];
            fprintf(stderr, "[ndfl] count chain %zu: %.2f ms, %u blocks, start %llu, %llu bits, %llu bytes, status %u\n",
                    idx[t], (r.pad >> 16) * 0.01, r.pad & 0xFFFFu, (unsigned long long)starts[idx[t]],
                    (unsigned long long)(r.end_bit - starts[idx[t]]), (unsigned long long)r.out_count, r.status);
        }
    }
    {
        float a = 0, b = 0;
        hipEventElapsedTime(&a, S.ev[0], S.ev[1]);
        hipEventElapsedTime(&b, S.ev[2], S.ev[3]);
        S.last_ms_find = a; S.last_ms_count = b;
    }

    const size_t n0 = starts.size();
    std::unordered_map<uint64_t, size_t> extra;
    auto find_at = [&](uint64_t b, size_t& idx) -> bool {
        auto it = std::lower_bound(starts.begin(), starts.begin() + n0, b);
        if (it != starts.begin() + n0 && *it == b) { idx = (size_t)(it - starts.begin()); return true; }
        auto e = extra.find(b);
        if (e != extra.end()) { idx = e->second; return true; }
        return false;
    };
    for (int round = 0; round < 8; round++) {
        std::vector<uint64_t> todo;
        size_t dummy;
        for (size_t k = 0; k < res.size(); k++)
            if (res[k].status == ST_BOUNDARY && res[k].end_bit < end_bit &&
                !(res[k].next < n0 && starts[res[k].next] == res[k].end_bit) && !find_at(res[k].end_bit, dummy)) {
                extra[res[k].end_bit] = NONE;
                todo.push_back(res[k].end_bit);
            }
        if (todo.empty()) break;
        std::vector<ChainRes> r2;
        rc = run_count(todo, r2);
        if (rc) return rc;
        for (size_t k = 0; k < todo.size(); k++) {
            starts.push_back(todo[k]);
            res.push_back(r2[k]);
            extra[todo[k]] = starts.size() - 1;
        }
        S.repairs += todo.size();
    }
    ht[2] = hnow();
    std::vector<EmitChain> chains;
    std::vector<uint64_t> offs;
    uint64_t off = dict_len;
    size_t cur = 0;
    uint64_t stop_bit = 0;
    for (;;) {
        const ChainRes& r = res[cur];
        EmitChain ec;
        ec.start_bit = starts[cur];
        ec.end_bit = r.end_bit;
        ec.out_off = off;
        ec.out_count = r.out_count;
        ec.slot = cur;
        chains.push_back(ec);
        offs.push_back(off);
        off += r.out_count;
        if (r.status == ST_FINAL) { stop_bit = r.end_bit; break; }
        if (r.status == ST_ERROR) break;
        if (r.end_bit == end_bit) { stop_bit = end_bit; break; }
        if (r.end_bit > end_bit) return -1;
        size_t nxt;
        if (r.next < n0 && starts[r.next] == r.end_bit) { cur = r.next; continue; }
        if (find_at(r.end_bit, nxt) && nxt != (size_t)NONE) { cur = nxt; continue; }
        std::vector<uint64_t> st1{r.end_bit};
        std::vector<ChainRes> r1;
        rc = run_count(st1, r1);
        if (rc) return rc;
        starts.push_back(r.end_bit);
        res.push_back(r1[0]);
        extra[r.end_bit] = starts.size() - 1;
        cur = starts.size() - 1;
        S.repairs++;
    }
    S.chains = chains.size();
    S.flat_chains = 0;
    S.candidates = sorted_cand.size();
    if (S.knobs.stats) {
        uint32_t st[SW_QCOUNT + 1] = {0};
        INF_CHK(hipMemcpy(st, S.d_stats, sizeof(st), hipMemcpyDeviceToHost));
        fprintf(stderr, "[ndfl] finder quick survivors %u; count pass: chains %zu candidates %zu repairs %llu "
                "slow-verify lanes %u fixups %u rounds %u\n", st[SW_QCOUNT], chains.size(), sorted_cand.size(),
                (unsigned long long)S.repairs, st[SW_NSLOW], st[SW_NFIX], st[SW_NROUND]);
        const int prc = print_count_stats(S, false);
        if (prc) return prc;
    }
    const uint64_t total = off - dict_len;
    ht[3] = hnow();
    if (total > out_cap) { *out_len = total; return -3; }

    const uint32_t nch = (uint32_t)chains.size();
    INF_CHK(inf_ensure(&S.d_chains, &S.d_chains_cap, nch * sizeof(EmitChain)));
    INF_CHK(inf_ensure(&S.d_res, &S.d_res_cap, nch * sizeof(ChainRes)));
    if (!S.d_ticket) INF_CHK(hipMalloc(&S.d_ticket, 64));
    INF_CHK(hipMemcpyAsync(S.d_chains, chains.data(), nch * sizeof(EmitChain), hipMemcpyHostToDevice, s));
    INF_CHK(hipMemsetAsync(S.d_ticket, 0, 64, s));
    uint8_t* d_out;
    const bool direct = (flags & 2u) != 0;
    if (direct) d_out = out;
    else {
        INF_CHK(inf_ensure(&S.d_out, &S.d_out_cap, dict_len + total + 64));
        d_out = (uint8_t*)S.d_out;
        if (dict_len) INF_CHK(hipMemcpyAsync(d_out, out, dict_len, hipMemcpyHostToDevice, s));
    }
    const uint64_t nbytes = dict_len + total;
    if ((nbytes + 31) / 32 > 0xFFFFFFFFull) return -2;
    const uint64_t npw = (nbytes + 31) / 32;
    INF_CHK(inf_ensure(&S.d_ref, &S.d_ref_cap, nbytes * 4 + 64));
    INF_CHK(inf_ensure(&S.d_pend, &S.d_pend_cap, npw * 4 + 64));
    INF_CHK(hipMemsetAsync(S.d_pend, 0, npw * 4 + 64, s));
    if (!S.h_cnt) INF_CHK(hipHostMalloc(&S.h_cnt, 64, 0));
    hipEvent_t e2 = S.ev[4], e3 = S.ev[5];
    INF_CHK(hipEventRecord(e2, s));
    if (!S.d_ph) INF_CHK(hipMalloc(&S.d_ph, (size_t)std::max(COUNT_WAVES, EMIT_WAVES) * sizeof(wv::PhArr)));
    static const uint32_t emit_grid = wave_grid(ndfl_inflate_emit_wave_kernel, EMIT_WAVES, "NDFL_EMIT_WPC");
    hipLaunchKernelGGL(ndfl_inflate_emit_wave_kernel, dim3(std::min<uint32_t>(nch, emit_grid)), dim3(64), 0, s, d_w,
                       nwords, nbits, (const EmitChain*)S.d_chains, nch, (uint32_t*)S.d_ticket, d_out,
                       (ChainRes*)S.d_res, (const uint64_t*)S.d_cands, ncand, (uint32_t*)S.d_ref, (uint32_t*)S.d_pend,
                       pool, (wv::PhArr*)S.d_ph, stats_on ? (uint32_t*)S.d_stats : nullptr, (const uint64_t*)nullptr,
                       (const uint32_t*)nullptr, (const uint32_t*)nullptr);
    INF_CHK(hipGetLastError());
    INF_CHK(hipEventRecord(e3, s));
    std::vector<ChainRes> er(nch);
    INF_CHK(hipMemcpyAsync(er.data(), S.d_res, nch * sizeof(ChainRes), hipMemcpyDeviceToHost, s));
    INF_CHK(hipStreamSynchronize(s));
    ht[4] = hnow();
    float ms = 0;
    hipEventElapsedTime(&ms, e2, e3);
    S.last_ms_emit = ms;
    if (stats_on) {
        uint64_t t64[48];
        INF_CHK(hipMemcpy(t64, (const uint32_t*)S.d_stats + SW_CLOCK64, sizeof(t64), hipMemcpyDeviceToHost));
        const double span = (double)(t64[17] - ~t64[18]);
        fprintf(stderr, "[ndfl] emit waves %llu: busy %.1f ms x waves, span %.3f ms, occupancy %.3f, longest chain %.3f ms\n",
                (unsigned long long)t64[19], t64[16] * 1e-5, span * 1e-5, t64[19] ? t64[16] / (span * t64[19]) : 0.0,
                t64[20] * 1e-5);
    }
    if (deferred) {
        S.pending = true;
        S.p_out = d_out; S.p_nbytes = nbytes; S.p_dict_len = dict_len;
    } else {
        uint64_t groups = 0;
        const int rr = resolve_rounds(S, s, d_out, nbytes, &groups);
        if (rr) return rr;
        S.resolved_groups = groups;
    }
    INF_CHK(hipEventRecord(e3, s));
    INF_CHK(hipStreamSynchronize(s));
    float ms2 = 0;
    hipEventElapsedTime(&ms2, S.ev[0], e3);
    S.last_ms_wall = ms2;
    hipEventElapsedTime(&ms2, e2, e3);
    *last_ms = ms2;
    ht[5] = hnow();
    if (htime) fprintf(stderr, "[ndfl] inflate host ms: finder+starts %.2f count+repairs %.2f link %.2f emit %.2f resolve %.2f\n",
                       ht[1] - ht[0], ht[2] - ht[1], ht[3] - ht[2], ht[4] - ht[3], ht[5] - ht[4]);
    for (uint32_t k = 0; k < nch; k++) {
        if (er[k].status == ST_ERROR) {
            if (partial && er[k].reason == R_UEOS) {
                const uint64_t produced = chains[k].out_off - dict_len + er[k].bnd_cnt;
                if (!direct && produced) INF_CHK(hipMemcpy(out + dict_len, d_out + dict_len, produced, hipMemcpyDeviceToHost));
                *out_len = produced;
                *consumed_bits = er[k].bnd_bit;
                return NEED_INPUT;
            }
            const uint64_t produced = chains[k].out_off - dict_len + er[k].out_count;
            if (!direct && produced) INF_CHK(hipMemcpy(out + dict_len, d_out + dict_len, produced, hipMemcpyDeviceToHost));
            *out_len = produced;
            *consumed_bits = er[k].end_bit;
            return (int)er[k].reason;
        }
    }
    if (!direct && total) INF_CHK(hipMemcpy(out + dict_len, d_out + dict_len, total, hipMemcpyDeviceToHost));
    *out_len = total;
    *consumed_bits = stop_bit;
    return 0;
}

static int inflate_sync(InflateScratch& S, hipStream_t s, const uint8_t* in, uint64_t in_len, uint64_t from_bit,
                        uint64_t window_bits, uint32_t flags, uint64_t* sync_bit, double* last_ms) {
    uint64_t olen = 0, bits = 0;
    const uint64_t end = std::min(in_len * 8, from_bit + window_bits);
    if (from_bit >= end) { *sync_bit = inf::NONE; return 0; }
    return inflate_run(S, s, in, in_len, from_bit, end, nullptr, 0, 0, &olen, &bits, flags, false, last_ms, false,
                       sync_bit);
}

constexpr uint32_t TAIL_STEPS = 4096;
extern "C" __global__ void __launch_bounds__(256)
ndfl_inflate_tail_kernel(const uint32_t* pend, const uint32_t* ref, const uint8_t* out, uint64_t t0, uint64_t n,
                         uint8_t* dst, uint32_t* fail) {
    const uint64_t k = (uint64_t)blockIdx.x * 256 + threadIdx.x;
    if (k >= n) return;
    uint64_t p = t0 + k;
    uint32_t steps = 0;
    while ((pend[p >> 5] >> (p & 31)) & 1) {
        p -= ref[p];
        if (++steps > TAIL_STEPS) { atomicOr(fail, 1u); return; }
    }
    dst[k] = out[p];
}

constexpr uint32_t TAIL_LITERAL = 0x80000000u;
extern "C" __global__ void __launch_bounds__(256)
ndfl_inflate_tail_map_kernel(const uint32_t* pend, const uint32_t* ref, const uint8_t* out, uint64_t t0, uint64_t n,
                             uint64_t dict_len, uint32_t* dst, uint32_t* fail) {
    const uint64_t k = (uint64_t)blockIdx.x * 256 + threadIdx.x;
    if (k >= n) return;
    uint64_t p = t0 + k;
    uint32_t steps = 0;
    while ((pend[p >> 5] >> (p & 31)) & 1) {
        p -= ref[p];
        if (++steps > TAIL_STEPS) { atomicOr(fail, 1u); return; }
    }
    dst[k] = p < dict_len ? (uint32_t)p : TAIL_LITERAL | out[p];
}

static int inflate_tail_map(InflateScratch& S, hipStream_t s, uint64_t n, uint32_t* dst) {
    if (!S.pending) return -5;
    if (n > S.p_nbytes) return -1;
    if (n == 0) return 0;
    if (!S.h_cnt) INF_CHK(hipHostMalloc(&S.h_cnt, 64, 0));
    uint32_t* d_fail = (uint32_t*)S.d_stats + SW_TAIL_FAIL;
    INF_CHK(hipMemsetAsync(d_fail, 0, 4, s));
    hipLaunchKernelGGL(ndfl_inflate_tail_map_kernel, dim3((uint32_t)((n + 255) / 256)), dim3(256), 0, s,
                       (const uint32_t*)S.d_pend, (const uint32_t*)S.d_ref, (const uint8_t*)S.p_out, S.p_nbytes - n, n,
                       S.p_dict_len, dst, d_fail);
    INF_CHK(hipGetLastError());
    uint32_t* h = (uint32_t*)S.h_cnt;
    INF_CHK(hipMemcpyAsync(h + 8, d_fail, 4, hipMemcpyDeviceToHost, s));
    INF_CHK(hipStreamSynchronize(s));
    return h[8] ? -6 : 0;
}

static int inflate_tail(InflateScratch& S, hipStream_t s, uint64_t n, uint8_t* dst) {
    if (!S.pending) return -5;
    if (n > S.p_nbytes) return -1;
    if (n == 0) return 0;
    if (!S.h_cnt) INF_CHK(hipHostMalloc(&S.h_cnt, 64, 0));
    uint32_t* d_fail = (uint32_t*)S.d_stats + SW_TAIL_FAIL;
    INF_CHK(hipMemsetAsync(d_fail, 0, 4, s));
    hipLaunchKernelGGL(ndfl_inflate_tail_kernel, dim3((uint32_t)((n + 255) / 256)), dim3(256), 0, s,
                       (const uint32_t*)S.d_pend, (const uint32_t*)S.d_ref, (const uint8_t*)S.p_out, S.p_nbytes - n, n,
                       dst, d_fail);
    INF_CHK(hipGetLastError());
    uint32_t* h = (uint32_t*)S.h_cnt;
    INF_CHK(hipMemcpyAsync(h + 8, d_fail, 4, hipMemcpyDeviceToHost, s));
    INF_CHK(hipStreamSynchronize(s));
    return h[8] ? -6 : 0;
}

static int inflate_resolve(InflateScratch& S, hipStream_t s, uint64_t* n_resolved) {
    using namespace inf;
    *n_resolved = 0;
    if (!S.pending) return -5;
    S.pending = false;
    const int rr = resolve_rounds(S, s, S.p_out, S.p_nbytes, n_resolved);
    if (rr) return rr;
    S.resolved_groups = *n_resolved;
    return 0;
}
```

deflate-library-java_amd/csrc/hip/inflate_wave.hpp:

```cpp
#pragma once

namespace wv {
using namespace inf;

enum : uint32_t { K_LIT = 0, K_LEN = 1, K_EOB = 2, K_BAD = 3 };

struct Shared {
    Tabs t;
    uint8_t lens[320];
    uint16_t cl_tab[128];
    uint32_t exit_[64];
    uint8_t kind_[64];
    uint64_t h_pos, h_d0;
    uint32_t h_err, h_bfinal, h_btype, h_len, h_numlit, h_numdist;
};

struct PhArr {
    uint32_t cp[7][64];
    uint32_t end[7][64];
    uint32_t cnt[7][64];
    uint8_t kr[7][64];
};

__device__ __forceinline__ uint32_t lit_entry(uint32_t sym, uint32_t len) {
// ... 995 lines not shown

__device__ __noinline__ void round_decode_phased(const In& in, const Tabs& t, bool ed, uint64_t rs, uint64_t E,
                                                 Shared& S, Stage& stg, int lane, Seg& out, uint32_t& first_term,
                                                 uint32_t& nfix, Geo& g, uint32_t esc4) {
    g = make_geo(in, rs, E);
    stage_round(in, g, stg, lane);
    const Lv v = make_lv(stg, g, lane);
    const uint32_t nb = g.nb;
    uint32_t s, e;
    lane_seg(g, lane, s, e);
    uint32_t endv[8], cntv[8], fbcv[8], krv[8];
    uint32_t fbl = 0, fbh = 0;
    constexpr uint32_t G = 2;
#pragma unroll 1
    for (uint32_t f = 0; f < 8; f += G) {
        PhOut P[G];
        if (esc4) phase_multi_esc<G>(v, t, ed, nb, s + f, e, esc4, P);
        else phase_multi<G>(v, t, ed, nb, s + f, e, P);
#pragma unroll
        for (uint32_t h = 0; h < G; h++) {
            const uint32_t g = f + h;
#pragma unroll
            for (uint32_t k = 0; k < 8; k++) {
                endv[k] = k == g ? P[h].end : endv[k];
                cntv[k] = k == g ? P[h].cnt : cntv[k];
                fbcv[k] = k == g ? P[h].fbc : fbcv[k];
                krv[k] = k == g ? P[h].kr : krv[k];
            }
            const uint32_t fo = (P[h].fb != NOCP && P[h].fb - s < 255u) ? P[h].fb - s : 255u;
            if (g < 4) fbl |= fo << (8 * g); else fbh |= fo << (8 * (g - 4));
        }
    }
    uint32_t Q = 0;
#pragma unroll
    for (uint32_t f = 0; f < 8; f++) {
        const uint32_t x = __shfl_up(endv[f], 1, 64);
        const uint32_t vv = phase_of(x - s, fbl, fbh) & 15u;
        if (lane > 0) Q |= vv << (4 * f);
    }
#pragma unroll
    for (int k = 1; k < 64; k <<= 1) {
        const uint32_t B = __shfl_up(Q, k, 64);
        if (lane >= k) Q = map_compose(Q, B);
    }
    const uint32_t myph = Q & 15u;
    const uint32_t xsel = myph < 8 ? sel8(endv, myph) : NOCP;
    uint32_t x = __shfl_up(xsel, 1, 64);
    if (lane == 0) x = s;
    SegR r;
    r.start = x; r.end = x; r.cnt = 0; r.kind = T_ERR; r.reason = R_INTERNAL;
    bool known = false;
    if (myph < 8) {
        const uint32_t pc = phase_of(x - s, fbl, fbh);
        const uint32_t f = pc & 15u;
        if (f == myph) {
            known = true;
            const uint32_t kr = sel8(krv, f);
            r.end = sel8(endv, f);
            r.cnt = sel8(cntv, f) - ((pc & 16u) ? sel8(fbcv, f) : 0u);
            r.kind = kr >> 5; r.reason = kr & 31u;
        }
    }
    const uint64_t km = __ballot(!known);
    const uint32_t u = km ? (uint32_t)__builtin_ctzll(km) : 64u;
    const uint64_t tm = __ballot(known && r.kind != T_EXIT);
    const uint32_t t0 = tm ? (uint32_t)__builtin_ctzll(tm) : 64u;
    first_term = min(t0, 64u);
    if (u < t0) {
        S.exit_[lane] = r.end;
        __syncthreads();
        first_term = 64;
        for (uint32_t j = u; j < 64 && first_term == 64; j++) {
            nfix++;
            if ((uint32_t)lane == j) {
                const uint32_t st = j ? (uint32_t)S.exit_[j - 1] : s;
                uint32_t en, cn, kr, fb, fbc;
                if (esc4) {
                    PhOut P1[1];
                    phase_multi_esc<1>(v, t, ed, nb, st, e, esc4, P1);
                    en = P1[0].end; cn = P1[0].cnt; kr = P1[0].kr;
                } else {
                    phase_run(v, t, ed, nb, st, e, en, cn, kr, fb, fbc);
                }
                r.start = st; r.end = en; r.cnt = cn; r.kind = kr >> 5; r.reason = kr & 31u;
                S.exit_[lane] = en;
                S.kind_[lane] = r.kind;
            }
            __syncthreads();
            if (S.kind_[j] != T_EXIT) first_term = j;
        }
    }
    out.start = g.base + r.start; out.end = g.base + r.end; out.cnt = r.cnt;
    out.kind = r.kind; out.reason = r.reason;
}

__device__ __forceinline__ uint64_t wave_sum_u64(uint64_t x) {
#pragma unroll
    for (int o = 32; o > 0; o >>= 1) x += __shfl_xor((unsigned long long)x, o, 64);
    return x;
}
__device__ __forceinline__ uint64_t wave_excl_u64(uint64_t v, int lane) {
    uint64_t x = v;
#pragma unroll
    for (int o = 1; o < 64; o <<= 1) {
        const uint64_t y = __shfl_up((unsigned long long)x, o, 64);
        if (lane >= o) x += y;
    }
    return x - v;
}

__device__ __forceinline__ bool is_cand(const uint64_t* cands, uint32_t ncand, uint64_t b, uint32_t* idx = nullptr) {
    uint32_t lo = 0, hi = ncand;
    while (lo < hi) { const uint32_t mid = (lo + hi) >> 1; if (cands[mid] < b) lo = mid + 1; else hi = mid; }
    if (idx) *idx = lo;
    return lo < ncand && cands[lo] == b;
}

__device__ __forceinline__ uint64_t next_cand(const uint64_t* cands, uint32_t ncand, uint64_t b, uint64_t limit) {
    uint32_t lo = 0, hi = ncand;
    while (lo < hi) { const uint32_t mid = (lo + hi) >> 1; if (cands[mid] <= b) lo = mid + 1; else hi = mid; }
    const uint64_t nx = lo < ncand ? cands[lo] : NONE;
    return min(nx, limit);
}

struct CandCur {
    const uint64_t* c;
    uint32_t n, i;
    uint64_t v;
    __device__ __forceinline__ void init(const uint64_t* cands, uint32_t ncand, uint64_t b) {
        c = cands; n = ncand;
        uint32_t lo = 0, hi = n;
        while (lo < hi) { const uint32_t mid = (lo + hi) >> 1; if (c[mid] < b) lo = mid + 1; else hi = mid; }
        i = lo;
        v = i < n ? c[i] : NONE;
    }
    __device__ __forceinline__ bool at(uint64_t b, uint32_t* idx) {
        while (v < b) { i++; v = i < n ? c[i] : NONE; }
        *idx = i;
        return v == b;
    }
    __device__ __forceinline__ uint64_t after(uint64_t b, uint64_t limit) {
        while (v <= b) { i++; v = i < n ? c[i] : NONE; }
        return min(v, limit);
    }
};

typedef __attribute__((address_space(1))) uint8_t gu8;
typedef __attribute__((address_space(1))) uint32_t gu32;
typedef __attribute__((address_space(1))) uint64_t gu64;

#ifdef NDFL_EMIT_NOSTORE
#define NDFL_OA(x) ((x) & 0xFFFull)
#else
#define NDFL_OA(x) (x)
#endif
typedef uint32_t u32x4v __attribute__((ext_vector_type(4)));
typedef __attribute__((address_space(1))) u32x4v gu128;
struct Wr {
    uint64_t acc;
    uint32_t an;
    uint64_t dst;
    uint32_t q0, q1, q2, hn;
};
__device__ __forceinline__ void wr_init(Wr& w, uint64_t dst) {
    w.acc = 0; w.an = 0; w.dst = dst;
    w.q0 = 0; w.q1 = 0; w.q2 = 0; w.hn = 0;
}
__device__ __forceinline__ void wr_drain(Wr& w, gu8* out) {
    if (w.hn) {
        gu8* d = out + NDFL_OA(w.dst - 4 * w.hn);
        if (w.hn >= 2) *(gu64*)d = (uint64_t)w.q0 | ((uint64_t)w.q1 << 32);
        if (w.hn == 1) *(gu32*)d = w.q0;
        if (w.hn == 3) *(gu32*)(d + 8) = w.q2;
        w.hn = 0;
    }
}
__device__ __forceinline__ void wr_lit(Wr& w, gu8* out, uint32_t val, uint32_t n) {
    w.acc |= (uint64_t)val << (8 * w.an);
    w.an += n;
    if (w.an >= 4) {
        const uint32_t word = (uint32_t)w.acc;
        if (w.hn == 3) {
            *(gu128*)(out + NDFL_OA(w.dst - 12)) = u32x4v{w.q0, w.q1, w.q2, word};
            w.hn = 0;
        } else {
            w.q0 = w.hn == 0 ? word : w.q0;
            w.q1 = w.hn == 1 ? word : w.q1;
            w.q2 = w.hn == 2 ? word : w.q2;
            w.hn++;
        }
        w.acc >>= 32;
        w.an -= 4;
        w.dst += 4;
    }
}
__device__ __forceinline__ void wr_flush_word(Wr& w, gu8* out) {
    wr_drain(w, out);
    if (w.an) {
        *(gu32*)(out + NDFL_OA(w.dst)) = (uint32_t)w.acc;
        w.dst += w.an;
        w.acc = 0;
        w.an = 0;
    }
}
__device__ __forceinline__ void wr_flush_exact(Wr& w, gu8* out) {
    wr_drain(w, out);
    for (uint32_t k = 0; k < w.an; k++) out[NDFL_OA(w.dst + k)] = (uint8_t)(w.acc >> (8 * k));
    w.dst += w.an;
    w.acc = 0;
    w.an = 0;
}
__device__ __forceinline__ void wrs_lit(Wr& w, gu8* out, uint32_t val, uint32_t n) {
    w.acc |= (uint64_t)val << (8 * w.an);
    w.an += n;
    const bool full = w.an >= 4;
    const uint32_t word = (uint32_t)w.acc;
    if (full && w.hn == 3) *(gu128*)(out + NDFL_OA(w.dst - 12)) = u32x4v{w.q0, w.q1, w.q2, word};
    w.q0 = full ? w.q1 : w.q0;
    w.q1 = full ? w.q2 : w.q1;
    w.q2 = full ? word : w.q2;
    w.hn = (w.hn + (full ? 1u : 0u)) & 3u;
    w.acc = full ? w.acc >> 32 : w.acc;
    w.an &= 3u;
    w.dst += full ? 4u : 0u;
}
__device__ __forceinline__ void wrs_drain(Wr& w, gu8* out) {
    if (w.hn) {
        gu8* d = out + NDFL_OA(w.dst - 4 * w.hn);
        if (w.hn == 1) *(gu32*)d = w.q2;
        if (w.hn == 2) *(gu64*)d = (uint64_t)w.q1 | ((uint64_t)w.q2 << 32);
        if (w.hn == 3) { *(gu64*)d = (uint64_t)w.q0 | ((uint64_t)w.q1 << 32); *(gu32*)(d + 8) = w.q2; }
        w.hn = 0;
    }
}
__device__ __forceinline__ void wrs_flush_word(Wr& w, gu8* out) {
    wrs_drain(w, out);
    if (w.an) {
        *(gu32*)(out + NDFL_OA(w.dst)) = (uint32_t)w.acc;
        w.dst += w.an;
        w.acc = 0;
        w.an = 0;
    }
}
__device__ __forceinline__ void wrs_flush_exact(Wr& w, gu8* out) {
    wrs_drain(w, out);
    for (uint32_t k = 0; k < w.an; k++) out[NDFL_OA(w.dst + k)] = (uint8_t)(w.acc >> (8 * k));
    w.dst += w.an;
    w.acc = 0;
    w.an = 0;
}
__device__ __forceinline__ uint64_t ld8(const gu8* p) { return *(const gu64*)p; }
__device__ __forceinline__ uint32_t ld4(const gu8* p) { return *(const gu32*)p; }
__device__ __forceinline__ void wr_copy(gu8* out, uint64_t dst, uint32_t len, uint32_t dist, uint32_t& lastb) {
    gu8* d = out + NDFL_OA(dst);
    const gu8* sp = out + NDFL_OA(dst - dist);
    if (dist == 1) {
        const uint32_t v4 = lastb * 0x01010101u;
        if (len >= 16) {
            const u32x4v x = {v4, v4, v4, v4};
            uint32_t k = 0;
            for (; k + 16 <= len; k += 16) *(gu128*)(d + k) = x;
            if (k < len) *(gu128*)(d + len - 16) = x;
            return;
        }
        if (len >= 4) {
            uint32_t k = 0;
            for (; k + 4 <= len; k += 4) *(gu32*)(d + k) = v4;
            if (k < len) *(gu32*)(d + len - 4) = v4;
        } else {
            for (uint32_t k = 0; k < len; k++) d[k] = (uint8_t)lastb;
        }
        return;
    }
    if (dist >= 16 && len >= 16) {
        uint32_t k = 0;
        u32x4v x = {0, 0, 0, 0};
        for (; k + 16 <= len; k += 16) { x = *(const gu128*)(sp + k); *(gu128*)(d + k) = x; }
        if (k < len) { x = *(const gu128*)(sp + len - 16); *(gu128*)(d + len - 16) = x; }
        lastb = x.w >> 24;
        return;
    }
    if (dist >= 8 && len >= 8) {
        uint32_t k = 0;
        uint64_t x = 0;
        for (; k + 8 <= len; k += 8) { x = ld8(sp + k); *(gu64*)(d + k) = x; }
        if (k < len) { x = ld8(sp + len - 8); *(gu64*)(d + len - 8) = x; }
        lastb = (uint32_t)(x >> 56);
        return;
    }
    if (dist >= 4 && len >= 4) {
        uint32_t k = 0, x = 0;
        for (; k + 4 <= len; k += 4) { x = ld4(sp + k); *(gu32*)(d + k) = x; }
        if (k < len) { x = ld4(sp + len - 4); *(gu32*)(d + len - 4) = x; }
        lastb = x >> 24;
        return;
    }
    uint32_t b = lastb;
    for (uint32_t k = 0; k < len; k++) { b = sp[k]; d[k] = (uint8_t)b; }
    lastb = b;
}

}

extern "C" __global__ void __launch_bounds__(64)
ndfl_inflate_hdr_kernel(const uint32_t* w, uint64_t nwords, uint64_t nbits, const uint64_t* cands, uint32_t ncand,
                        wv::HdrRec* rec, uint32_t* flat_list, uint32_t* nflat, uint32_t* flat_flag) {
    using namespace wv;
    __shared__ __attribute__((aligned(16))) uint32_t lens[64][80];
    __shared__ uint16_t clt[64][128];
    __shared__ uint32_t win[8 * 64];
    const uint32_t lane = threadIdx.x;
    const uint32_t k = blockIdx.x * 64 + lane;
    if (k >= ncand) return;
    const In in{w, nwords, nbits};
    for (uint32_t q = 0; q < 80; q++) lens[lane][q] = 0;
    const uint64_t p = cands[k];
    Hdr h;
    parse_hdr_core<RdWin>(in, p, (uint8_t*)lens[lane], clt[lane], h, win + lane);
    HdrRec* r = rec + k;
    for (uint32_t q = 0; q < 80; q += 4)
        *(uint4*)&r->lens[q] = make_uint4(lens[lane][q], lens[lane][q + 1], lens[lane][q + 2], lens[lane][q + 3]);
    r->h = h;
    r->at = p;
    uint32_t c8 = 0;
    bool bad = false;
    for (uint32_t q = 0; q < 72; q++) {
        const uint32_t v = lens[lane][q];
#pragma unroll
        for (uint32_t b = 0; b < 4; b++) {
            const uint32_t l = (v >> (8 * b)) & 0xFFu;
            c8 += l == 8 ? 1u : 0u;
            bad = bad || (l - 1u < 7u) || (l == 8 && q >= 64);
        }
    }
    const uint32_t esc = 256u - min(c8, 256u);
    const uint32_t kk = esc == 1 ? 1u : esc == 2 ? 2u : esc == 4 ? 3u : 0u;
    r->flat = (flat_list && h.err == 0 && h.btype == 2 && !bad) ? kk : 0u;
    r->pad = 0;
    if (flat_flag) flat_flag[k] = r->flat;
    if (flat_list) {
        const uint64_t m = __ballot(r->flat != 0);
        uint32_t b = 0;
        if (lane == 0 && m) b = atomicAdd(nflat, (uint32_t)__popcll(m));
        b = __shfl(b, 0, 64);
        if (r->flat) flat_list[b + (uint32_t)__popcll(m & ((1ull << lane) - 1ull))] = k;
    }
}

#ifndef NDFL_COUNT_WPE
#define NDFL_COUNT_WPE 3
#endif
namespace wv {
#ifndef NDFL_FLAT_OTHER_MAX
#define NDFL_FLAT_OTHER_MAX 64
#endif
#ifndef NDFL_FLAT_K
#define NDFL_FLAT_K 4
#endif
#ifndef NDFL_FLAT_PRIO
#define NDFL_FLAT_PRIO 1
#endif
#ifdef NDFL_FLAT_PROF
__device__ unsigned long long g_flat_prof[4];
#endif
constexpr uint32_t FLAT_ESC_WORD = 64;
static_assert(FLAT_ESC_WORD + 64 * 64 / 4 <= SW * 64, "flat escape tables in the stage");

__device__ __forceinline__ uint32_t flat_esc_entry(const TabsG& t, uint32_t kk, uint32_t x) {
    const uint32_t pl = 8 - kk;
    const uint32_t w = ((1u << pl) - 1u) | (x << pl);
    uint32_t e = t.lit[w & ((1u << LB) - 1u)];
    uint32_t len, kind;
    if (e >> 31) {
        len = e & 15; kind = 0;
    } else {
        if (!(e & 31)) e = long_lit(e, w, t);
        len = e & 31;
        const uint32_t k = (e >> 9) & 3;
        kind = k == K_LIT ? 0u : k == K_EOB ? 1u : 2u;
    }
    return (kind < 2 && len > pl && len <= pl + 6) ? (len | (kind << 4)) : 0u;
}

__device__ __forceinline__ uint32_t count_flat_group(const In& in, const uint32_t* flist, uint32_t n,
                                                     const uint64_t* cands, uint32_t ncand, uint64_t limit,
                                                     uint64_t stop_all, ChainRes* res, const SegPool& pool,
                                                     const HdrRec* hrec, Shared& S, uint32_t* stw, int lane,
                                                     uint32_t* redo, uint32_t& tb_next, uint32_t& tb_end,
                                                     uint32_t* whys) {
    lu8* escs = (lu8*)((lu32*)stw + FLAT_ESC_WORD);
    uint32_t my_c = 0, my_brec = NOREC, my_kk = 0;
    uint64_t my_d0 = 0;
    bool my_ok = false, my_final = false, my_ed = false;
    for (uint32_t k = 0; k < n; k++) {
        const uint32_t c = flist[k];
        const HdrRec* hr = hrec + c;
        uint32_t* lw = (uint32_t*)S.lens;
        lw[lane] = hr->lens[lane];
        if (lane < 16) lw[64 + lane] = hr->lens[64 + lane];
        if (lane == 0) hdr_to_shared(hr->h, S);
        const uint32_t kk = hr->flat - 1u;
        __syncthreads();
        bool ed;
        const int te = build_tables(S, lane, ed, stw);
        uint32_t brec = NOREC;
        if (!te) {
            if (c < pool.nslot && pool.nbt) {
                brec = claim_table_record(pool, tb_next, tb_end, lane);
                if (brec != NOREC)
                    write_table_record(pool, brec, S.t, cands[c], S.h_d0, S.h_bfinal, S.h_btype, ed,
                                       ((1u << (8 - kk)) - 1u) * 0x01010101u,
                                       (uint32_t)lane, 64);
            }
            const TabsG tg{S.t.lit, S.t.dst, S.t.lx, S.t.dx};
            escs[k * 64 + lane] = (uint8_t)flat_esc_entry(tg, kk, (uint32_t)lane);
        }
        if ((uint32_t)lane == k) {
            my_c = c; my_ok = !te; my_d0 = S.h_d0; my_final = S.h_bfinal != 0; my_ed = ed; my_brec = brec; my_kk = kk;
        }
        __syncthreads();
    }
    const bool active = (uint32_t)lane < n && my_ok;
    uint32_t ci = my_c;
    uint64_t cv = active ? cands[ci] : NONE;
    auto after = [&](uint64_t b) {
        while (cv <= b) { ci++; cv = ci < ncand ? cands[ci] : NONE; }
        return min(cv, limit);
    };
    uint32_t nr = 0;
    if (active) {
        const uint64_t e0 = after(my_d0);
        nr = (uint32_t)min<uint64_t>((e0 > my_d0 ? (e0 - my_d0 + MAX_SPAN - 1) / MAX_SPAN : 1) + 1, 1024);
    }
    uint64_t cv1 = NONE, cv2 = NONE, cv3 = NONE;
    if (active) {
        cv1 = ci + 1 < ncand ? cands[ci + 1] : NONE;
        cv2 = ci + 2 < ncand ? cands[ci + 2] : NONE;
        cv3 = ci + 3 < ncand ? cands[ci + 3] : NONE;
    }
    const uint32_t rpre = (uint32_t)wave_excl_u64(nr, lane), rtot = (uint32_t)wave_sum_u64(nr);
    uint32_t rb = 0;
    if (lane == 0 && rtot) rb = atomicAdd(pool.ctr, rtot);
    rb = __builtin_amdgcn_readfirstlane(rb);
    bool ok = false;
    uint64_t total = 0, endpos = 0;
    uint32_t status = ST_BOUNDARY, next_idx = 0xFFFFFFFFu, why = active ? 4u : 5u;
    if (active) {
        const uint32_t pl = 8 - my_kk, M4 = ((1u << pl) - 1u) * 0x01010101u;
        bool recording = my_c < pool.nslot;
        uint32_t rnext = rb + rpre, rlast = rnext + nr;
        uint32_t brec = my_brec, others = 0;
        const uint64_t o64 = (my_d0 >> 8) << 8;
        const uint64_t og4 = o64 >> 7;
        const uint32_t nbo = (uint32_t)min<uint64_t>(in.nbits - min(in.nbits, o64), 0xFFFFFF00ull);
        uint32_t pos = (uint32_t)(my_d0 - o64);
        lu32* ring = (lu32*)&S.t + lane;
        uint32_t fw = (pos >> 5) & ~7u;
#pragma unroll
        for (uint32_t i = 0; i < 24; i += 4) {
            const u32x4 v = in.ld4(og4 + ((fw + i) >> 2));
            ring[i * 64] = v.x; ring[(i + 1) * 64] = v.y; ring[(i + 2) * 64] = v.z; ring[(i + 3) * 64] = v.w;
        }
        fw += 24;
        uint32_t frow = 0;
        u32x4 ra = in.ld4(og4 + (fw >> 2)), rb = in.ld4(og4 + (fw >> 2) + 1);
        uint32_t base = 0, r0 = 0, re = 0, per = 0, pw = 0, nbr = 0, idx = NOREC, j = 0, p = 0, jst = 0, bytes = 0, sn = 0;
        uint64_t* ps = nullptr;
        uint32_t* pc = nullptr;
        SegMeta* mp = nullptr;
        uint32_t* link = pool.head + my_c;
        uint32_t st = 0;
        if (NDFL_FLAT_PRIO) __builtin_amdgcn_s_setprio(3);
        auto end_round = [&](bool eob) {
            if (ps) {
                const uint64_t ex = o64 + base + p;
                ps[j] = o64 + base + jst;
                pc[j] = bytes;
                for (uint32_t jj = j + 1; jj < 64; jj++) { ps[jj] = ex; pc[jj] = 0; }
                uint32_t kf = eob ? (uint32_t)T_EOB : (uint32_t)T_EXIT;
                asm volatile("" : "+v"(kf));
                write_round_meta(mp, eob ? j : 64u, kf, 0u, NOREC, ex, ex, pw, brec, o64 + base + r0);
                *link = idx;
                link = &mp->next;
                brec = NOREC;
            }
            total += bytes;
            pos = base + p;
        };
#ifdef NDFL_FLAT_PROF
        unsigned long long fp_ph = 0, fp_t0 = clock64(), fp_n = 0;
#endif
        while (st < 2) {
            {
#ifdef NDFL_FLAT_PROF
                const unsigned long long fp_a = clock64();
#endif
                const uint32_t cw = (st == 1 ? base + p : pos) >> 5;
                if (cw + 16 >= fw) {
                    ring[frow * 64] = ra.x; ring[(frow + 1) * 64] = ra.y; ring[(frow + 2) * 64] = ra.z;
                    ring[(frow + 3) * 64] = ra.w; ring[(frow + 4) * 64] = rb.x; ring[(frow + 5) * 64] = rb.y;
                    ring[(frow + 6) * 64] = rb.z; ring[(frow + 7) * 64] = rb.w;
                    fw += 8;
                    frow = frow == 16 ? 0u : frow + 8;
                    ra = in.ld4(og4 + (fw >> 2)); rb = in.ld4(og4 + (fw >> 2) + 1);
                }
#ifdef NDFL_FLAT_PROF
                asm volatile("s_waitcnt lgkmcnt(0)" ::: "memory");
                fp_ph += clock64() - fp_a;
                fp_n++;
#endif
            }
            for (uint32_t k = 0; k < NDFL_FLAT_K && st < 2; k++) {
                if (st == 0) {
                    const uint64_t rsa = o64 + pos;
                    if (cv <= rsa) { cv = cv1; cv1 = cv2; cv2 = cv3; cv3 = NONE; ci++; }
                    if (cv <= rsa) {
                        while (cv <= rsa) { ci++; cv = ci < ncand ? cands[ci] : NONE; }
                        cv1 = ci + 1 < ncand ? cands[ci + 1] : NONE;
                        cv2 = ci + 2 < ncand ? cands[ci + 2] : NONE;
                        cv3 = ci + 3 < ncand ? cands[ci + 3] : NONE;
                    }
                    uint64_t E = min(min(cv, limit), rsa + MAX_SPAN);
                    if (E <= rsa) E = rsa + 1;
                    base = pos & ~31u;
                    r0 = pos - base; re = (uint32_t)(E - o64) - base;
                    pw = seg_pw(re - r0); per = pw * 32;
                    nbr = nbo - min(nbo, base);
                    idx = NOREC;
                    if (recording) {
                        if (rnext >= rlast) {
                            rnext = atomicAdd(pool.ctr, 8u);
                            rlast = rnext + 8;
                        }
                        if (rnext < pool.nrec) idx = rnext++;
                        else recording = false;
                    }
                    ps = idx != NOREC ? pool.start + (uint64_t)idx * 64 : nullptr;
                    pc = idx != NOREC ? pool.cnt + (uint64_t)idx * 64 : nullptr;
                    mp = idx != NOREC ? pool.meta + idx : nullptr;
                    j = 0; p = r0; jst = r0; bytes = 0;
                    sn = seg_end(r0, per, re, 0);
                    st = 1;
                }
                if (st != 1) continue;
                const uint32_t ap = base + p, cw = ap >> 5;
                const bool tk_ok = p < sn && cw + 2 < fw;
                uint32_t rr0 = frow + 24 - min(fw - cw, 24u);
                rr0 = rr0 >= 24 ? rr0 - 24 : rr0;
                const uint32_t rr1 = rr0 == 23 ? 0u : rr0 + 1, rr2 = rr1 == 23 ? 0u : rr1 + 1;
                const uint32_t w0 = ring[rr0 * 64], w1 = ring[rr1 * 64], w2 = ring[rr2 * 64];
                const uint32_t sh = ap & 31u;
                const uint32_t lo = __builtin_amdgcn_alignbit(w1, w0, sh), hi = __builtin_amdgcn_alignbit(w2, w1, sh);
                uint32_t ln;
                asm volatile("v_mbcnt_lo_u32_b32 %0, -1, 0\n\tv_mbcnt_hi_u32_b32 %0, -1, %0" : "=v"(ln));
                const uint32_t ent = escs[ln * 64 + ((lo >> pl) & 63u)], len = ent & 15u;
                const uint32_t q = (sn - min(sn, p) + 7) >> 3, qi = (nbr - min(nbr, p)) >> 3;
                const uint32_t t = tk_ok ? min(min(esc_index(lo, hi, M4), q), qi) : 0u;
                const bool esc = tk_ok && t == 0 && (lo & (M4 & 0xFFu)) == (M4 & 0xFFu) && ent && p + len <= nbr;
                const bool eob = esc && (ent >> 4);
                p += t ? 8 * t : esc ? len : 0u;
                bytes += t ? t : (esc && !eob) ? 1u : 0u;
                bool ended = eob;
                if (tk_ok && t == 0 && !esc) {
                    if (my_brec == NOREC || ++others > NDFL_FLAT_OTHER_MAX) {
                        st = 3; why = 2;
                    } else {
                        const TabsG tg = tabs_view(tabrec(pool, my_brec));
                        uint32_t pp = 0;
                        Tok tk;
                        tok_e<true>(lo, hi, tg.lit[lo & ((1u << LB) - 1u)], pp, tg, my_ed, sn - p, nbr - min(nbr, p), tk);
                        if (tk.kind == K_LIT || tk.kind == K_LEN) bytes += tk.n;
                        else if (tk.kind == K_EOB) ended = true;
                        else { st = 3; why = 3; }
                        p += pp;
                    }
                    ended = ended || st == 3;
                }
                const bool rend = !ended && p >= sn && j == 63;
                if (ended || rend) {
                    if (st != 3) { end_round(!rend); st = rend ? 0u : 2u; }
                } else {
                    const bool sw = p >= sn;
                    if (sw && ps) { ps[j] = o64 + base + jst; pc[j] = bytes; }
                    total += sw ? bytes : 0u;
                    j += sw ? 1u : 0u;
                    jst = sw ? p : jst;
                    bytes = sw ? 0u : bytes;
                    sn = sw ? seg_end(r0, per, re, j) : sn;
                }
            }
        }
        if (NDFL_FLAT_PRIO) __builtin_amdgcn_s_setprio(0);
#ifdef NDFL_FLAT_PROF
        if (lane == 0) {
            atomicAdd(&g_flat_prof[0], clock64() - fp_t0); atomicAdd(&g_flat_prof[1], fp_ph); atomicAdd(&g_flat_prof[2], fp_n);
        }
#endif
        if (st == 2) {
            const uint64_t cur = o64 + pos;
            if (my_final) { status = ST_FINAL; endpos = cur; ok = true; }
            else if (cur >= stop_all) { status = ST_BOUNDARY; endpos = cur; ok = true; }
            else {
                while (cv < cur) { ci++; cv = ci < ncand ? cands[ci] : NONE; }
                next_idx = ci;
                if (cv == cur) { status = ST_BOUNDARY; endpos = cur; ok = true; }
            }
        }
    }
    if (ok) {
        ChainRes o;
        o.end_bit = endpos; o.out_count = total; o.status = status; o.reason = 0; o.next = next_idx; o.pad = 0;
        o.bnd_bit = 0; o.bnd_cnt = 0;
        res[my_c] = o;
    }
    const bool rd = (uint32_t)lane < n && !ok;
    if (whys && rd) atomicAdd(&whys[why], 1u);
// ... 466 lines not shown
    const uint32_t nlist = (uint32_t)info[LI_NCH];
    const In in{w, nwords, nbits};
    for (;;) {
    uint32_t tk0 = 0;
    if (lane == 0) tk0 = atomicAdd(ticket, 1u);
    const uint32_t t = __builtin_amdgcn_readfirstlane(tk0);
    if (t >= nlist) break;
    const uint32_t ci = eorder[t];
    const EmitChain ch = chains[ci];
    uint64_t cur = ch.start_bit, base = ch.out_off;
    uint32_t status = ST_BOUNDARY, reason = 0;
    uint64_t endpos = ch.start_bit;
    bool abort = false;
    uint32_t rec = ch.slot < pool.nslot ? pool.head[ch.slot] : NOREC;
    SegMeta pm = {};
    uint64_t pst = 0;
    uint32_t pcn = 0;
    rec_fetch(pool, rec, lane, pm, pst, pcn);
    uint64_t bnd_bit = cur, bnd_out = base;
    for (int blk = 0;; blk++) {
        if (blk > 0 && cur == ch.end_bit) { status = ST_BOUNDARY; endpos = cur; break; }
        bnd_bit = cur; bnd_out = base;
        if (cur + 3 > nbits) { abort = true; break; }
        const uint32_t hb = (uint32_t)(in.win64(cur)) & 7u;
        if ((hb >> 1) == 0) {
            const uint64_t hp = (cur + 3 + 7) & ~7ull;
            if (hp + 32 > nbits) { abort = true; break; }
            const uint32_t lw = (uint32_t)in.win64(hp);
            if ((lw >> 16) != (~lw & 0xFFFFu)) { abort = true; break; }
            const uint64_t ln = lw & 0xFFFFu, d0 = hp + 32;
            if (d0 + 8 * ln > nbits) { abort = true; break; }
            const uint64_t ib = d0 >> 3;
            for (uint64_t i = (uint64_t)lane; i < ln; i += 64) {
                const uint64_t b = ib + i;
                out[base + i] = (uint8_t)(in.ld(b >> 2) >> (8 * (uint32_t)(b & 3)));
            }
            base += ln;
            cur = d0 + 8 * ln;
            if (hb & 1) { status = ST_FINAL; endpos = cur; break; }
            continue;
        }
        const TabRec* btr = block_tables(pool, rec, pm, cur);
        if (!btr) { abort = true; break; }
        __syncthreads();
        {
            static_assert(offsetof(Tabs, lit) == 0 && offsetof(Tabs, dst) == sizeof(Tp) - sizeof(btr->t.dst), "primary tables first");
            const uint4* src = (const uint4*)&btr->t;
            uint4* dst = (uint4*)Tp;
            for (uint32_t q = (uint32_t)lane; q < sizeof(Tp) / 16; q += 64) dst[q] = src[q];
            const TabsG tv = tabs_view(btr);
            T.lx = tv.lx;
            T.dx = tv.dx;
        }
        const bool bfinal = btr->bfinal != 0, ed = btr->ed != 0;
        const uint32_t tph = btr->phase;
        const bool ph8 = tph != TP_NONE;
        const uint32_t esc4 = tph > TP_LIT8 ? tph : 0u;
        __syncthreads();
        bool block_done = false, chain_done = false;
        while (!block_done) {
            if (rec == NOREC) { abort = true; chain_done = true; break; }
            const SegMeta m = pm;
            const uint32_t ft = m.ft;
            const uint64_t rstart = pst;
            const uint32_t rcnt = pcn;
            rec = m.next;
            rec_fetch(pool, rec, lane, pm, pst, pcn);
            uint64_t rend;
            uint32_t kind, rsn;
            round_lane_end(m, rstart, lane, rend, kind, rsn);
            const Geo g = make_geo(in, m.rs, m.rs + 1, m.pw);
            const bool live = (uint32_t)lane <= ft;
            const uint64_t mycnt = live ? rcnt : 0ull;
            const uint64_t pre = wave_excl_u64(mycnt, lane);
            const uint64_t rsum = wave_sum_u64(mycnt);
            stage_round(in, g, stg, lane);
            const Lv v = make_lv(stg, g, lane);
            const uint32_t nb = g.nb;
            uint32_t pos = (uint32_t)(rstart - g.base);
            uint32_t end = (uint32_t)(rend - g.base);
            const uint64_t dst0 = base + pre;
            uint32_t n = 0;
            Wr wr;
            wr_init(wr, dst0);
            uint64_t dfr = ~0ull, lastsrc = 0;
            bool lsp = false;
            uint32_t lastb = 0;
            bool lastok = false;
            Bb bb;
            const uint32_t lim = min(end, nb - min(nb, 48u));
            bool fast = live && pos < lim;
            if (fast) bb_init(bb, v, pos);
            auto token_loop = [&](auto ph) {
                using PH = decltype(ph);
                while (live && pos < end) {
                    if (fast) {
#pragma unroll 1
                        for (uint32_t k = 0; k < NDFL_EMITF_LITRUN_K; k++) {
                            if (PH::value && bb.pos >= lim) break;
                            if (PH::value && esc4) {
                                const uint32_t lo = (uint32_t)bb.buf, hi = (uint32_t)(bb.buf >> 32);
                                const uint32_t t = min(min(esc_index(lo, hi, esc4), bb.nb >> 3), (end - bb.pos + 7) >> 3);
                                if (t) {
                                    uint32_t b[8];
#pragma unroll
                                    for (uint32_t i = 0; i < 8; i++)
                                        b[i] = (T.lit[(i < 4 ? lo >> (8 * i) : hi >> (8 * (i - 4))) & 0xFFu] >> 9) & 0xFFu;
                                    const uint32_t v0 = b[0] | (b[1] << 8) | (b[2] << 16) | (b[3] << 24);
                                    const uint32_t v1 = b[4] | (b[5] << 8) | (b[6] << 16) | (b[7] << 24);
                                    const uint32_t n0 = min(t, 4u);
                                    wrs_lit(wr, gout, n0 == 4 ? v0 : v0 & ((1u << (8 * n0)) - 1u), n0);
                                    if (t > 4) wrs_lit(wr, gout, t == 8 ? v1 : v1 & ((1u << (8 * (t - 4))) - 1u), t - 4);
                                    lastb = ((t > 4 ? (v1 >> (8 * (t - 5))) & 0xFFu : (v0 >> (8 * (t - 1))) & 0xFFu) << 9);
                                    bb.buf = t < 8 ? bb.buf >> (8 * t) : 0ull;
                                    bb.nb -= 8 * t;
                                    bb.pos += 8 * t;
                                    bb_refill(bb, v);
                                    continue;
                                }
                            }
                            if (PH::value && !esc4 && bb.nb >= 34 && bb.pos + 24 < end) {
                                const uint32_t lo = (uint32_t)bb.buf, hi = (uint32_t)(bb.buf >> 32);
                                const uint32_t e0 = T.lit[lo & ((1u << LB) - 1u)], e1 = T.lit[(lo >> 8) & ((1u << LB) - 1u)];
                                const uint32_t e2 = T.lit[(lo >> 16) & ((1u << LB) - 1u)];
                                const uint32_t e3 = T.lit[__builtin_amdgcn_alignbit(hi, lo, 24) & ((1u << LB) - 1u)];
                                if (((e0 & 0x800001FFu) == 0x80000088u) && ((e1 & 0x800001FFu) == 0x80000088u) &&
                                    ((e2 & 0x800001FFu) == 0x80000088u) && ((e3 & 0x800001FFu) == 0x80000088u)) {
                                    wrs_lit(wr, gout, ((e0 >> 9) & 0xFFu) | (((e1 >> 9) & 0xFFu) << 8) | (((e2 >> 9) & 0xFFu) << 16) | (((e3 >> 9) & 0xFFu) << 24), 4);
                                    lastb = e3;
                                    bb_skip(bb, 32);
                                    bb_refill(bb, v);
                                    continue;
                                }
                            }
                            const uint32_t e = T.lit[(uint32_t)bb.buf & ((1u << LB) - 1u)];
                            if (!((e >> 31) && bb.pos + 2u * LB < lim)) break;
                            wrs_lit(wr, gout, (e >> 9) & 0xFFFFu, 1u + ((e >> 8) & 1u));
                            lastb = e;
                            bb_skip(bb, e & 15);
                            bb_refill(bb, v);
                        }
                        pos = bb.pos;
                        const uint32_t nn = (uint32_t)(wr.dst - dst0) + wr.an;
                        if (nn != n) {
                            lsp = true;
                            lastb = (lastb >> ((lastb >> 8) & 1u ? 17 : 9)) & 0xFFu;
                            lastok = true;
                            n = nn;
                        }
                        if (PH::value) {
                            fast = pos < lim;
                            if (pos >= end) break;
                        }
                    }
                    Tok tk;
                    if (fast) {
                        tok_bb<true>(bb, v, T, ed, tk, end);
                        pos = bb.pos;
                        fast = pos < lim;
                    } else {
                        tok<true>(v, pos, T, ed, end, nb, tk);
                    }
                    if (tk.kind == K_LIT) {
                        wrs_lit(wr, gout, tk.val, tk.n);
                        n += tk.n;
                        lsp = true;
                        lastb = tk.val >> (tk.n == 2 ? 8 : 0);
                        lastok = true;
                        continue;
                    }
                    if (tk.kind != K_LEN) break;
                    const uint64_t dst = dst0 + n;
                    if ((uint64_t)tk.dist > dst) { kind = T_ERR; rsn = R_COPY_BEFORE; end = pos; break; }
                    const uint32_t len = tk.n, dist = tk.dist;
                    const uint64_t src = dst - dist;
                    const uint64_t src_end = src + min(len, dist);
                    bool defer = src < dst0;
                    if (!defer && src_end > dfr) {
                        for (uint64_t q = src >> 5; q <= (src_end - 1) >> 5 && !defer; q++) {
                            const uint64_t lo = max(src, q << 5), hi = min(src_end, (q + 1) << 5);
                            const uint32_t mk = (uint32_t)(((1ull << (hi - lo)) - 1) << (lo & 31));
                            defer = (__hip_atomic_load(&pend[q], __ATOMIC_RELAXED, __HIP_MEMORY_SCOPE_AGENT) & mk) != 0;
                        }
                    }
                    wrs_flush_word(wr, gout);
                    if (!defer && dist == 1 && !lastok) lastb = gout[dst - 1];
                    if (!defer) {
                        wr_copy(gout, dst, len, dist, lastb);
                        lastok = true;
                        lsp = true;
                    } else {
                        const uint64_t anchor = dist == 1 ? (n > 0 ? (lsp ? dst - 1 : lastsrc) : src) : 0;
                        for (uint32_t k = 0; k < len; k++) {
                            const uint64_t back = dst + k - anchor;
                            ref[dst + k] = dist == 1 ? (back < (1ull << 32) ? (uint32_t)back : 1u) : dist;
                        }
                        for (uint64_t q = dst >> 5; q <= (dst + len - 1) >> 5; q++) {
                            const uint64_t lo = max(dst, q << 5), hi = min(dst + len, (q + 1) << 5);
                            const uint32_t mk = (uint32_t)(((1ull << (hi - lo)) - 1) << (lo & 31));
                            atomicOr(&pend[q], mk);
                        }
                        lastsrc = anchor;
                        lsp = dist != 1;
                        dfr = min(dfr, dst);
                        lastok = false;
                    }
                    n += len;
                    wr.dst = dst0 + n;
                }
            };
            if (ph8) token_loop(std::true_type{}); else token_loop(std::false_type{});
            wrs_flush_exact(wr, gout);
            if (live && kind != T_ERR && (n != rcnt || pos != end)) { kind = T_ERR; rsn = R_INTERNAL; }
            const uint64_t em = __ballot(live && kind == T_ERR);
            if (em) {
                const int fl = (int)__builtin_ctzll(em);
                status = ST_ERROR;
                reason = __shfl(rsn, fl, 64);
                endpos = g.base + __shfl(end, fl, 64);
                base = __shfl((unsigned long long)(dst0 + n), fl, 64);
                chain_done = true;
                break;
            }
            base += rsum;
            if (ft < 64) {
                block_done = true;
                cur = __shfl((unsigned long long)rend, (int)ft, 64);
                if (bfinal) { status = ST_FINAL; endpos = cur; chain_done = true; }
            }
        }
        if (chain_done) break;
    }
    if (lane == 0) {
        if (abort) {
            slow[atomicAdd(nslow, 1u)] = ci;
        } else {
            ChainRes o;
            o.end_bit = endpos; o.out_count = base - ch.out_off; o.status = status; o.reason = reason;
            o.next = 0xFFFFFFFFu; o.pad = 0;
            o.bnd_bit = bnd_bit; o.bnd_cnt = bnd_out - ch.out_off;
            res[ci] = o;
        }
    }
    }
}

#ifndef NDFL_RESOLVE_HOPS
#define NDFL_RESOLVE_HOPS 4
#endif
extern "C" __global__ void __launch_bounds__(256)
ndfl_inflate_resolve_kernel(const uint32_t* list, const uint32_t* nlist, const uint32_t* pend, uint32_t* ref,
                            uint8_t* out, uint32_t* newbits) {
    const uint32_t n = *nlist;
    const uint32_t b = threadIdx.x & 31;
    for (uint32_t k = (blockIdx.x * 256 + threadIdx.x) >> 5; k < n; k += gridDim.x * 8) {
        const uint64_t wd = list[k];
        const uint32_t bits = pend[wd];
        bool still = false;
        if ((bits >> b) & 1) {
            const uint64_t i = wd * 32 + b;
            uint64_t d = ref[i];
            uint64_t p = i - d;
            bool pending = (pend[p >> 5] >> (p & 31)) & 1;
#pragma unroll 1
            for (int h = 1; h < NDFL_RESOLVE_HOPS && pending; h++) {
                const uint64_t nd = d + ref[p];
                if (nd >= (1ull << 32)) break;
                d = nd;
                p = i - d;
                pending = (pend[p >> 5] >> (p & 31)) & 1;
            }
            if (pending) {
                const uint64_t nd = d + ref[p];
                ref[i] = (uint32_t)(nd < (1ull << 32) ? nd : d);
                still = true;
            } else {
                out[i] = out[p];
            }
        }
        const uint64_t m = __ballot(still);
        if (b == 0) newbits[k] = (uint32_t)(m >> (threadIdx.x & 32));
    }
}

__device__ __forceinline__ void block_append(bool flag, uint32_t v, uint32_t* list, uint32_t* n) {
    __shared__ uint32_t wc[4], wbase;
    const int lane = threadIdx.x & 63, wid = threadIdx.x >> 6;
    const uint64_t m = __ballot(flag);
    if (lane == 0) wc[wid] = (uint32_t)__popcll(m);
    __syncthreads();
    if (threadIdx.x == 0) {
        const uint32_t t = wc[0] + wc[1] + wc[2] + wc[3];
        wbase = t ? atomicAdd(n, t) : 0u;
    }
    __syncthreads();
    uint32_t off = wbase;
    for (int k = 0; k < wid; k++) off += wc[k];
    if (flag) list[off + __popcll(m & ((1ull << lane) - 1))] = v;
    __syncthreads();
}

extern "C" __global__ void __launch_bounds__(256)
ndfl_inflate_resolve_apply_kernel(const uint32_t* list, const uint32_t* nlist, uint32_t* pend, const uint32_t* newbits,
                                  uint32_t* list_out, uint32_t* nlist_out, uint32_t* nbytes_out) {
    const uint32_t n = *nlist;
    for (uint32_t k0 = blockIdx.x * 256; k0 < n; k0 += gridDim.x * 256) {
        const uint32_t k = k0 + threadIdx.x;
        const bool live = k < n;
        uint32_t nb = 0, wd = 0;
        if (live) { wd = list[k]; nb = newbits[k]; pend[wd] = nb; }
        if (nbytes_out) {
            const uint32_t c = wave_sum((uint32_t)__popc(nb));
            if ((threadIdx.x & 63) == 0 && c) atomicAdd(nbytes_out, c);
        }
        block_append(live && nb != 0, wd, list_out, nlist_out);
    }
}

extern "C" __global__ void __launch_bounds__(256)
ndfl_inflate_pending_list_kernel(const uint32_t* pend, uint64_t w0, uint64_t w1, uint32_t* list, uint32_t* nlist) {
    __shared__ uint32_t sh[4], sbase;
    const uint64_t base = w0 + ((uint64_t)blockIdx.x * 256 + threadIdx.x) * 16;
    uint32_t v[16];
    if (base + 16 <= w1 && (base & 3) == 0) {
        const u32x4* q = (const u32x4*)(pend + base);
#pragma unroll
        for (int k = 0; k < 4; k++) { const u32x4 x = q[k]; v[4 * k] = x.x; v[4 * k + 1] = x.y; v[4 * k + 2] = x.z; v[4 * k + 3] = x.w; }
    } else {
#pragma unroll
        for (int k = 0; k < 16; k++) v[k] = base + k < w1 ? pend[base + k] : 0u;
    }
    uint32_t cnt = 0;
#pragma unroll
    for (int k = 0; k < 16; k++) cnt += v[k] != 0;
    uint32_t tot;
    const uint32_t off = block_excl_scan<uint32_t, 4>(cnt, sh, tot);
    if (threadIdx.x == 0) sbase = tot ? atomicAdd(nlist, tot) : 0u;
    __syncthreads();
    uint32_t o = sbase + off;
#pragma unroll
    for (int k = 0; k < 16; k++)
        if (v[k]) list[o++] = (uint32_t)(base + k);
}
```

Baseline: 228,500.

## Consolidate control buffers, fold memsets and copies into kernels, double link jumps

Merges stats, info and ticket buffers into one allocation cleared by a single memset, and drops several small memsets and device-to-device copies by having kernels zero the next counter or write flags directly. It also skips clearing the pending bitmap when the previous call left it clean, trims the pending-list scan to the produced output length, and halves the pointer-jumping launches by advancing two levels per kernel. Separately, it shrinks the header kernel to 32 active lanes per block to cut shared memory use. The aim is fewer stream operations and launches on the inflate path, at the cost of more complex buffer-state tracking and error-index encoding.

```diff
diff --git a/deflate-library-java_amd/csrc/hip/inflate_kernels.hip b/deflate-library-java_amd/csrc/hip/inflate_kernels.hip
--- a/deflate-library-java_amd/csrc/hip/inflate_kernels.hip
+++ b/deflate-library-java_amd/csrc/hip/inflate_kernels.hip
@@ -748,7 +748,10 @@
 
 constexpr uint32_t OB_NB = 24;
 constexpr uint32_t OB_WORDS = 2 * OB_NB;
-constexpr size_t CTK_BYTES = 512;
+constexpr uint32_t CT_FIRST = 16 + 2 * OB_WORDS;
+constexpr uint32_t CT_EMIT_TICKET = 128;
+constexpr uint32_t CT_RESOLVE = 144;
+constexpr size_t CTK_BYTES = 640;
 
 template <class Bk>
 __device__ __forceinline__ void border_count(Bk bk, uint32_t n, uint32_t* ob) {
@@ -822,8 +825,9 @@
 }
 extern "C" __global__ void __launch_bounds__(SCAN_T)
 ndfl_inflate_order_kernel(const uint64_t* cands, uint32_t n, uint64_t end_bit, uint32_t* order, const uint32_t* rep,
-                          uint32_t* nord, uint32_t* ob, const uint32_t* flat) {
+                          uint32_t* nord, uint32_t* ob, const uint32_t* flat, const uint32_t* nflat, uint64_t* nflat_out) {
     border_place(OrderBucket{cands, n, end_bit, rep, flat}, n, ob, order, nord);
+    if (nflat_out && blockIdx.x == 0 && threadIdx.x == 0) *nflat_out = *nflat;
 }
 
 struct EmitBucket {
@@ -858,12 +862,17 @@
     }
 }
 extern "C" __global__ void __launch_bounds__(256)
-ndfl_inflate_link_jump_kernel(const uint32_t* J, uint32_t* J2, const uint64_t* S, uint64_t* S2, const uint32_t* D,
-                              uint32_t* D2, uint32_t n) {
+ndfl_inflate_link_jump4_kernel(const uint32_t* J, uint32_t* J1, uint32_t* J2, const uint64_t* S, uint64_t* S2,
+                               const uint32_t* D, uint32_t* D2, uint32_t n) {
     for (uint32_t k = blockIdx.x * 256 + threadIdx.x; k < n; k += gridDim.x * 256) {
-        const uint32_t j = J[k];
-        if (j != NOLINK) { J2[k] = J[j]; S2[k] = S[k] + S[j]; D2[k] = D[k] + D[j]; }
-        else { J2[k] = NOLINK; S2[k] = S[k]; D2[k] = D[k]; }
+        uint64_t sum = S[k];
+        uint32_t d = D[k];
+        const uint32_t a = J[k];
+        uint32_t b = NOLINK, c = NOLINK, e = NOLINK;
+        if (a != NOLINK) { sum += S[a]; d += D[a]; b = J[a]; }
+        if (b != NOLINK) { sum += S[b]; d += D[b]; c = J[b]; }
+        if (c != NOLINK) { sum += S[c]; d += D[c]; e = J[c]; }
+        J1[k] = b; J2[k] = e; S2[k] = sum; D2[k] = d;
     }
 }
 extern "C" __global__ void __launch_bounds__(256)
@@ -908,14 +917,14 @@
     for (uint32_t k = 0; k < SCAN_PER; k++) st[k] = er[min(i0 + k, nch - 1)].status;
 #pragma unroll
     for (uint32_t k = 0; k < SCAN_PER; k++)
-        if (i0 + k < nch && st[k] == ST_ERROR) { atomicMin(first, i0 + k); break; }
+        if (i0 + k < nch && st[k] == ST_ERROR) { atomicMax(first, NOLINK - (i0 + k)); break; }
 }
 extern "C" __global__ void __launch_bounds__(64)
 ndfl_inflate_summary_kernel(const ChainRes* er, const EmitChain* chains, uint64_t* info, uint64_t dict_len,
                             uint32_t partial, const uint32_t* firstp) {
     using namespace inf;
     if (threadIdx.x != 0) return;
-    const uint32_t first = *firstp;
+    const uint32_t first = NOLINK - *firstp;
     if (first == NOLINK) {
         info[LI_CODE] = 0; info[LI_OUTLEN] = info[LI_TOTAL]; info[LI_CONSUMED] = info[LI_STOP];
         return;
@@ -933,7 +942,8 @@
 }
 
 #include "inflate_records.hpp"
-static_assert((CT_ORDER + 2 * OB_WORDS + 1) * 4 <= CTK_BYTES, "ticket buffer layout");
+static_assert(CT_FIRST == CT_ORDER + 2 * OB_WORDS && CT_FIRST < CT_EMIT_TICKET && CT_EMIT_TICKET + 9 <= CT_RESOLVE &&
+              (CT_RESOLVE + 3) * 4 <= CTK_BYTES, "ticket buffer layout");
 #include "inflate_wave.hpp"
 #include "inflate_wg.hpp"
 
@@ -955,6 +965,7 @@
     void* d_stops = nullptr; size_t d_stops_cap = 0;
     void* d_res = nullptr; size_t d_res_cap = 0;
     void* d_cands = nullptr; size_t d_cands_cap = 0;
+    void* d_ctl = nullptr;
     void* d_stats = nullptr;
     void* d_q = nullptr; size_t d_q_cap = 0;
     void* d_seg = nullptr; size_t d_seg_cap = 0;
@@ -963,6 +974,7 @@
     void* d_off = nullptr; size_t d_off_cap = 0;
     void* d_ref = nullptr; size_t d_ref_cap = 0;
     void* d_pend = nullptr; size_t d_pend_cap = 0;
+    size_t pend_dirty = 0;
     void* d_rl = nullptr; size_t d_rl_cap = 0;
     void* d_ticket = nullptr;
     void* d_slow = nullptr; size_t d_slow_cap = 0;
@@ -988,21 +1000,21 @@
     uint8_t* p_out = nullptr;
     uint64_t p_nbytes = 0, p_dict_len = 0;
     void release() {
-        void** ps[] = {&d_in, &d_cand, &d_starts, &d_stops, &d_res, &d_cands, &d_stats, &d_q, &d_seg, &d_chains, &d_off,
-                       &d_ref, &d_pend, &d_rl, &d_ticket, &d_ph, &d_cticket, &d_out, &d_hrec, &d_slow, &d_rep};
+        void** ps[] = {&d_in, &d_cand, &d_starts, &d_stops, &d_res, &d_cands, &d_ctl, &d_q, &d_seg, &d_chains, &d_off,
+                       &d_ref, &d_pend, &d_rl, &d_ticket, &d_ph, &d_out, &d_hrec, &d_slow, &d_rep};
         for (void** p : ps) { if (*p) hipFree(*p); *p = nullptr; }
+        d_stats = d_info = d_cticket = nullptr;
         for (auto& e : ev) { if (e) hipEventDestroy(e); e = nullptr; }
         if (h_cnt) hipHostFree(h_cnt);
         h_cnt = nullptr;
         if (h_info) hipHostFree(h_info);
         h_info = nullptr;
-        if (d_info) hipFree(d_info);
-        d_info = nullptr;
         if (d_link) hipFree(d_link);
         d_link = nullptr; d_link_cap = 0;
         d_in_cap = d_cand_cap = d_starts_cap = d_stops_cap = d_res_cap = d_cands_cap = d_seg_cap = d_q_cap = d_chains_cap = 0;
         d_off_cap = d_ref_cap = d_pend_cap = d_rl_cap = d_out_cap = d_hrec_cap = 0;
         pending = false;
+        pend_dirty = 0;
     }
 };
 
@@ -1062,6 +1074,29 @@
         return -4; } } while (0)
 #define INF_RC(x) do { const int _r = (x); if (_r) return _r; } while (0)
 
+constexpr size_t CTL_STATS_BYTES = 512, CTL_INFO_BYTES = LI_WORDS * 8;
+constexpr size_t CTL_BYTES = CTL_STATS_BYTES + CTL_INFO_BYTES + CTK_BYTES;
+static int ctl_ensure(InflateScratch& S) {
+    if (S.d_ctl) return 0;
+    INF_CHK(hipMalloc(&S.d_ctl, CTL_BYTES));
+    S.d_stats = S.d_ctl;
+    S.d_info = (char*)S.d_ctl + CTL_STATS_BYTES;
+    S.d_cticket = (char*)S.d_info + CTL_INFO_BYTES;
+    return 0;
+}
+
+static int pend_prepare(InflateScratch& S, hipStream_t s, uint64_t npw) {
+    const size_t need = npw * 4 + 64;
+    if (!S.d_pend || need > S.d_pend_cap) {
+        INF_CHK(inf_ensure(&S.d_pend, &S.d_pend_cap, need));
+        S.pend_dirty = S.d_pend_cap;
+    }
+    if (S.pend_dirty) INF_CHK(hipMemsetAsync(S.d_pend, 0, S.pend_dirty, s));
+    S.pend_dirty = need;
+    return 0;
+}
+static void pend_clean(InflateScratch& S) { S.pend_dirty = 0; }
+
 static int resolve_rounds(InflateScratch& S, hipStream_t s, uint8_t* d_out, uint64_t nbytes, uint64_t* groups) {
     using namespace inf;
     *groups = 0;
@@ -1076,7 +1111,7 @@
     uint32_t* ref = (uint32_t*)S.d_ref;
     INF_CHK(hipMemsetAsync(cnt, 0, 8, s));
     hipLaunchKernelGGL(ndfl_inflate_pending_list_kernel, dim3((uint32_t)((npw + 4095) / 4096)), dim3(256), 0, s,
-                       (const uint32_t*)pend, (uint64_t)0, npw, lst[0], cnt);
+                       (const uint32_t*)pend, (uint64_t)0, npw, lst[0], cnt, (const uint64_t*)nullptr, (uint64_t)0);
     INF_CHK(hipGetLastError());
     if (!S.h_cnt) INF_CHK(hipHostMalloc(&S.h_cnt, 64, 0));
     uint32_t* h = (uint32_t*)S.h_cnt;
@@ -1102,7 +1137,8 @@
         INF_CHK(hipGetLastError());
         hipLaunchKernelGGL(ndfl_inflate_resolve_apply_kernel, dim3((uint32_t)std::min<uint64_t>(1024, (n + 255) / 256)),
                            dim3(256), 0, s, (const uint32_t*)lst[cur], (const uint32_t*)(cnt + cur), pend,
-                           (const uint32_t*)nb, lst[cur ^ 1], cnt + (cur ^ 1), rstats ? cnt + 2 + (cur ^ 1) : (uint32_t*)nullptr);
+                           (const uint32_t*)nb, lst[cur ^ 1], cnt + (cur ^ 1), rstats ? cnt + 2 + (cur ^ 1) : (uint32_t*)nullptr,
+                           (uint32_t*)nullptr);
         INF_CHK(hipGetLastError());
         cur ^= 1;
     }
@@ -1149,37 +1185,35 @@
     return 0;
 }
 
-static int resolve_rounds_dev(InflateScratch& S, hipStream_t s, uint8_t* d_out, uint64_t nbytes, int rounds,
-                              uint32_t** left, uint64_t* first_count_dst) {
+constexpr uint32_t DEV_ROUNDS = 6;
+constexpr uint32_t LI_LEFT = LI_WORDS - 1, LI_PEND0 = LI_WORDS - 3;
+static int resolve_rounds_dev(InflateScratch& S, hipStream_t s, uint8_t* d_out, uint64_t nbytes, uint64_t dict_len,
+                              bool first_count) {
     using namespace inf;
     const uint64_t npw = (nbytes + 31) / 32;
-    *left = nullptr;
     if (npw == 0) return 0;
     if (npw > 0xFFFFFFFFull) return -2;
     INF_CHK(inf_ensure(&S.d_rl, &S.d_rl_cap, npw * 12 + 64));
-    uint32_t* cnt = (uint32_t*)S.d_rl;
+    uint64_t* info = (uint64_t*)S.d_info;
+    uint32_t* cnt = (uint32_t*)S.d_cticket + CT_RESOLVE;
     uint32_t* lst[2] = {(uint32_t*)((char*)S.d_rl + 64), (uint32_t*)((char*)S.d_rl + 64) + npw};
     uint32_t* nb = lst[1] + npw;
     uint32_t* pend = (uint32_t*)S.d_pend;
     uint32_t* ref = (uint32_t*)S.d_ref;
-    INF_CHK(hipMemsetAsync(cnt, 0, 8, s));
     hipLaunchKernelGGL(ndfl_inflate_pending_list_kernel, dim3((uint32_t)((npw + 4095) / 4096)), dim3(256), 0, s,
-                       (const uint32_t*)pend, (uint64_t)0, npw, lst[0], cnt);
+                       (const uint32_t*)pend, (uint64_t)0, npw, lst[0], cnt, (const uint64_t*)(info + LI_TOTAL), dict_len);
     INF_CHK(hipGetLastError());
-    if (first_count_dst) INF_CHK(hipMemcpyAsync(first_count_dst, cnt, 4, hipMemcpyDeviceToDevice, s));
-    int cur = 0;
-    for (int round = 0; round < rounds; round++) {
-        INF_CHK(hipMemsetAsync(cnt + (cur ^ 1), 0, 4, s));
-        hipLaunchKernelGGL(ndfl_inflate_resolve_kernel, dim3(4096), dim3(256), 0, s, (const uint32_t*)lst[cur],
-                           (const uint32_t*)(cnt + cur), (const uint32_t*)pend, ref, d_out, nb);
+    if (first_count) INF_CHK(hipMemcpyAsync(info + LI_PEND0, cnt, 4, hipMemcpyDeviceToDevice, s));
+    for (uint32_t r = 0; r < DEV_ROUNDS; r++) {
+        uint32_t* n_out = r + 1 < DEV_ROUNDS ? cnt + (r + 1) % 3 : (uint32_t*)(info + LI_LEFT);
+        hipLaunchKernelGGL(ndfl_inflate_resolve_kernel, dim3(4096), dim3(256), 0, s, (const uint32_t*)lst[r & 1],
+                           (const uint32_t*)(cnt + r % 3), (const uint32_t*)pend, ref, d_out, nb);
         INF_CHK(hipGetLastError());
-        hipLaunchKernelGGL(ndfl_inflate_resolve_apply_kernel, dim3(1024), dim3(256), 0, s, (const uint32_t*)lst[cur],
-                           (const uint32_t*)(cnt + cur), pend, (const uint32_t*)nb, lst[cur ^ 1], cnt + (cur ^ 1),
-                           (uint32_t*)nullptr);
+        hipLaunchKernelGGL(ndfl_inflate_resolve_apply_kernel, dim3(1024), dim3(256), 0, s, (const uint32_t*)lst[r & 1],
+                           (const uint32_t*)(cnt + r % 3), pend, (const uint32_t*)nb, lst[(r + 1) & 1], n_out,
+                           (uint32_t*)nullptr, cnt + (r + 2) % 3);
         INF_CHK(hipGetLastError());
-        cur ^= 1;
-    }
-    *left = cnt + cur;
+    }
     return 0;
 }
 
@@ -1192,11 +1226,10 @@
                            uint64_t end_bit, uint8_t* out, uint64_t dict_len, uint64_t out_cap, uint64_t* out_len,
                            uint64_t* consumed_bits, uint32_t flags, bool deferred, bool partial, double* last_ms) {
     using namespace inf;
-    if (!S.d_info) INF_CHK(hipMalloc(&S.d_info, LI_WORDS * 8));
-    if (!S.h_info) INF_CHK(hipHostMalloc(&S.h_info, LI_WORDS * 8, 0));
+    if (!S.h_info) INF_CHK(hipHostMalloc(&S.h_info, CTL_STATS_BYTES + CTL_INFO_BYTES, 0));
     uint64_t* info = (uint64_t*)S.d_info;
-    volatile uint64_t* hinfo = (volatile uint64_t*)S.h_info;
-    INF_CHK(hipMemsetAsync(info, 0, LI_WORDS * 8, s));
+    volatile uint32_t* hstats = (volatile uint32_t*)S.h_info;
+    volatile uint64_t* hinfo = (volatile uint64_t*)((char*)S.h_info + CTL_STATS_BYTES);
     const uint64_t cap_all = (uint64_t)nseg * SEG_CAP + 1;
     const uint32_t ntile = (nseg + SCAN_TILE - 1) / SCAN_TILE;
     INF_CHK(inf_ensure(&S.d_starts, &S.d_starts_cap, (cap_all + nseg + 2 + ntile) * 8));
@@ -1224,10 +1257,9 @@
                            dim3(256), 0, s, (const uint64_t*)S.d_cands, info, d_w, nwords, nbits, d_rep);
         INF_CHK(hipGetLastError());
     }
-    INF_CHK(hipMemcpyAsync((void*)hinfo, info, (LI_NREP + 1) * 8, hipMemcpyDeviceToHost, s));
-    hinfo[LI_QCOUNT] = 0;
-    INF_CHK(hipMemcpyAsync((void*)(hinfo + LI_QCOUNT), (const uint32_t*)S.d_stats + SW_QCOUNT, 4, hipMemcpyDeviceToHost, s));
+    INF_CHK(hipMemcpyAsync((void*)hstats, S.d_stats, CTL_STATS_BYTES + (LI_NREP + 1) * 8, hipMemcpyDeviceToHost, s));
     INF_CHK(hipStreamSynchronize(s));
+    hinfo[LI_QCOUNT] = hstats[SW_QCOUNT];
     if ((uint32_t)hinfo[LI_QCOUNT] > S.q_cap && !S.q_full) { S.q_min = (uint32_t)hinfo[LI_QCOUNT] + 65536; return FIND_OVERFLOW; }
     const uint64_t n = hinfo[LI_NCAND];
     const uint64_t nrep = alias_on ? hinfo[LI_NREP] : n;
@@ -1242,8 +1274,6 @@
     INF_CHK(inf_ensure(&S.d_stops, &S.d_stops_cap, n * 12));
     INF_CHK(inf_ensure(&S.d_res, &S.d_res_cap, n * sizeof(ChainRes)));
     uint32_t* d_order = (uint32_t*)((char*)S.d_stops + n * 8);
-    if (!S.d_cticket) INF_CHK(hipMalloc(&S.d_cticket, CTK_BYTES));
-    INF_CHK(hipMemsetAsync(S.d_cticket, 0, CTK_BYTES, s));
     uint32_t* d_nord = (uint32_t*)S.d_cticket + CT_NORD;
     uint32_t* d_nflat = (uint32_t*)S.d_cticket + CT_NFLAT;
     uint32_t* d_ob = (uint32_t*)S.d_cticket + CT_ORDER;
@@ -1260,7 +1290,7 @@
         INF_CHK(inf_ensure(&S.d_hrec, &S.d_hrec_cap, (size_t)ncand * (sizeof(wv::HdrRec) + 8) + 64));
         d_flist = (uint32_t*)((char*)S.d_hrec + (size_t)ncand * sizeof(wv::HdrRec));
         d_fflag = d_flist + ncand;
-        hipLaunchKernelGGL(ndfl_inflate_hdr_kernel, dim3((ncand + 63) / 64), dim3(64), 0, s, d_w, nwords, nbits,
+        hipLaunchKernelGGL(ndfl_inflate_hdr_kernel, dim3((ncand + NDFL_HDR_LANES - 1) / NDFL_HDR_LANES), dim3(64), 0, s, d_w, nwords, nbits,
                            (const uint64_t*)S.d_cands, ncand, (wv::HdrRec*)S.d_hrec, flat_on ? d_flist : nullptr,
                            d_nflat, flat_on ? d_fflag : nullptr);
         INF_CHK(hipGetLastError());
@@ -1270,9 +1300,9 @@
     INF_CHK(hipGetLastError());
     hipLaunchKernelGGL(ndfl_inflate_order_kernel, dim3(otiles), dim3(SCAN_T), 0, s, (const uint64_t*)S.d_cands, ncand,
                        end_bit, d_order, (const uint32_t*)d_rep, (alias_on || flat_on) ? d_nord : (uint32_t*)nullptr, d_ob,
-                       flat_on ? (const uint32_t*)d_fflag : nullptr);
+                       flat_on ? (const uint32_t*)d_fflag : nullptr, (const uint32_t*)d_nflat,
+                       flat_on ? info + LI_NFLAT : (uint64_t*)nullptr);
     INF_CHK(hipGetLastError());
-    if (flat_on) INF_CHK(hipMemcpyAsync(info + LI_NFLAT, d_nflat, 4, hipMemcpyDeviceToDevice, s));
     launch_count(s, W, ncand,
                        d_w, nwords, nbits, (const uint64_t*)S.d_cands, (const uint64_t*)nullptr, ncand,
                        (const uint64_t*)S.d_cands, ncand, limit, (ChainRes*)S.d_res,
@@ -1349,10 +1379,10 @@
     }
     uint32_t nlev = 1;
     while ((1ull << nlev) < n) nlev++;
-    const size_t link_bytes = (size_t)(nlev + 1) * n * 4 + 2 * n * 8 + 2 * n * 4 + 64;
+    const size_t link_bytes = (size_t)(nlev + 2) * n * 4 + 2 * n * 8 + 2 * n * 4 + 64;
     INF_CHK(inf_ensure(&S.d_link, &S.d_link_cap, link_bytes));
     uint32_t* J = (uint32_t*)S.d_link;
-    uint64_t* Ssum[2] = {(uint64_t*)(((uintptr_t)(J + (size_t)(nlev + 1) * n) + 7) & ~(uintptr_t)7), nullptr};
+    uint64_t* Ssum[2] = {(uint64_t*)(((uintptr_t)(J + (size_t)(nlev + 2) * n) + 7) & ~(uintptr_t)7), nullptr};
     Ssum[1] = Ssum[0] + n;
     uint32_t* Dd[2] = {(uint32_t*)(Ssum[1] + n), nullptr};
     Dd[1] = Dd[0] + n;
@@ -1361,10 +1391,10 @@
                        (const uint64_t*)S.d_cands, end_bit, J, Ssum[0], Dd[0]);
     INF_CHK(hipGetLastError());
     int cur = 0;
-    for (uint32_t r = 0; r < nlev; r++) {
-        hipLaunchKernelGGL(ndfl_inflate_link_jump_kernel, dim3(lg), dim3(256), 0, s, (const uint32_t*)(J + (size_t)r * n),
-                           J + (size_t)(r + 1) * n, (const uint64_t*)Ssum[cur], Ssum[cur ^ 1], (const uint32_t*)Dd[cur],
-                           Dd[cur ^ 1], ncand);
+    for (uint32_t r = 0; r < nlev; r += 2) {
+        hipLaunchKernelGGL(ndfl_inflate_link_jump4_kernel, dim3(lg), dim3(256), 0, s, (const uint32_t*)(J + (size_t)r * n),
+                           J + (size_t)(r + 1) * n, J + (size_t)(r + 2) * n, (const uint64_t*)Ssum[cur], Ssum[cur ^ 1],
+                           (const uint32_t*)Dd[cur], Dd[cur ^ 1], ncand);
         INF_CHK(hipGetLastError());
         cur ^= 1;
     }
@@ -1397,10 +1427,8 @@
     if ((nbytes + 31) / 32 > 0xFFFFFFFFull) return LINK_FALLBACK;
     const uint64_t npw = (nbytes + 31) / 32;
     INF_CHK(inf_ensure(&S.d_ref, &S.d_ref_cap, nbytes * 4 + 64));
-    INF_CHK(inf_ensure(&S.d_pend, &S.d_pend_cap, npw * 4 + 64));
-    INF_CHK(hipMemsetAsync(S.d_pend, 0, npw * 4 + 64, s));
-    if (!S.d_ticket) INF_CHK(hipMalloc(&S.d_ticket, 64));
-    INF_CHK(hipMemsetAsync(S.d_ticket, 0, 64, s));
+    INF_RC(pend_prepare(S, s, npw));
+    uint32_t* tk = (uint32_t*)S.d_cticket + CT_EMIT_TICKET;
     if (S.knobs.test_segflip && S.pool.cnt) {
         uint32_t c0 = 0;
         INF_CHK(hipMemcpyAsync(&c0, S.pool.cnt, 4, hipMemcpyDeviceToHost, s));
@@ -1413,7 +1441,6 @@
     static const uint32_t emit_grid = wave_grid(ndfl_inflate_emit_wave_kernel, EMIT_WAVES, "NDFL_EMIT_WPC");
     if (S.knobs.emit_fast) {
         INF_CHK(inf_ensure(&S.d_slow, &S.d_slow_cap, (size_t)ncand * 4 + 64));
-        uint32_t* tk = (uint32_t*)S.d_ticket;
         static const uint32_t fast_grid = wave_grid(ndfl_inflate_emit_fast_kernel, EMIT_WAVES, "NDFL_EMITF_WPC");
         hipLaunchKernelGGL(ndfl_inflate_emit_fast_kernel, dim3(std::min<uint32_t>(ncand, fast_grid)), dim3(64), 0, s, d_w,
                            nwords, nbits, (const EmitChain*)S.d_chains, tk, d_out, (ChainRes*)S.d_res,
@@ -1434,7 +1461,7 @@
         }
     } else {
         hipLaunchKernelGGL(ndfl_inflate_emit_wave_kernel, dim3(std::min<uint32_t>(ncand, emit_grid)), dim3(64), 0, s, d_w,
-                           nwords, nbits, (const EmitChain*)S.d_chains, ncand, (uint32_t*)S.d_ticket, d_out,
+                           nwords, nbits, (const EmitChain*)S.d_chains, ncand, tk, d_out,
                            (ChainRes*)S.d_res, (const uint64_t*)S.d_cands, ncand, (uint32_t*)S.d_ref, (uint32_t*)S.d_pend,
                            S.pool, (wv::PhArr*)S.d_ph, stats_on ? (uint32_t*)S.d_stats : nullptr, (const uint64_t*)info,
                            (const uint32_t*)d_order, (const uint32_t*)nullptr);
@@ -1442,8 +1469,7 @@
     }
     INF_CHK(hipEventRecord(S.ev[5], s));
     {
-        uint32_t* d_first = (uint32_t*)S.d_cticket + CT_ORDER + 2 * OB_WORDS;
-        INF_CHK(hipMemsetAsync(d_first, 0xFF, 4, s));
+        uint32_t* d_first = (uint32_t*)S.d_cticket + CT_FIRST;
         hipLaunchKernelGGL(ndfl_inflate_first_error_kernel, dim3((ncand + SCAN_TILE - 1) / SCAN_TILE), dim3(SCAN_T), 0, s,
                            (const ChainRes*)S.d_res, (const uint64_t*)info, d_first);
         INF_CHK(hipGetLastError());
@@ -1451,11 +1477,9 @@
                            (const EmitChain*)S.d_chains, info, dict_len, partial ? 1u : 0u, (const uint32_t*)d_first);
         INF_CHK(hipGetLastError());
     }
-    uint32_t* left = nullptr;
     if (!deferred) {
-        rc = resolve_rounds_dev(S, s, d_out, nbytes, 6, &left, stats_on ? info + LI_WORDS - 3 : (uint64_t*)nullptr);
+        rc = resolve_rounds_dev(S, s, d_out, nbytes, dict_len, stats_on);
         if (rc) return rc;
-        if (left) INF_CHK(hipMemcpyAsync(info + LI_WORDS - 1, left, 4, hipMemcpyDeviceToDevice, s));
     }
     INF_CHK(hipMemcpyAsync((void*)hinfo, info, LI_WORDS * 8, hipMemcpyDeviceToHost, s));
     INF_CHK(hipStreamSynchronize(s));
@@ -1464,8 +1488,8 @@
         INF_CHK(hipMemcpy(st, S.d_stats, sizeof(st), hipMemcpyDeviceToHost));
         fprintf(stderr, "[ndfl] device link: chains %llu of %u candidates; count pass: slow-verify lanes %u fixups %u "
                 "rounds %u\n", (unsigned long long)hinfo[LI_NCH], ncand, st[SW_NSLOW], st[SW_NFIX], st[SW_NROUND]);
-        fprintf(stderr, "[ndfl] emit: %u pending 32-byte groups before the resolve rounds, %u after six\n",
-                (uint32_t)(hinfo[LI_WORDS - 3] & 0xFFFFFFFFu), (uint32_t)(hinfo[LI_WORDS - 1] & 0xFFFFFFFFu));
+        fprintf(stderr, "[ndfl] emit: %u pending 32-byte groups before the resolve rounds, %u after the device's\n",
+                (uint32_t)(hinfo[LI_PEND0] & 0xFFFFFFFFu), (uint32_t)(hinfo[LI_LEFT] & 0xFFFFFFFFu));
         rc = print_count_stats(S, true);
         if (rc) return rc;
     }
@@ -1477,7 +1501,7 @@
     S.flat_chains = hinfo[LI_NFLAT];
     S.repairs = 0;
     if (lflags & LF_CAPACITY) { *out_len = hinfo[LI_TOTAL]; return -3; }
-    const uint32_t pending_left = (uint32_t)(hinfo[LI_WORDS - 1] & 0xFFFFFFFFu);
+    const uint32_t pending_left = (uint32_t)(hinfo[LI_LEFT] & 0xFFFFFFFFu);
     S.pending_after_dev = deferred ? 0 : pending_left;
     if (!deferred && pending_left) {
         uint64_t groups = 0;
@@ -1499,6 +1523,7 @@
     S.last_ms_wall = w;
     *last_ms = w;
     const int code = (int)hinfo[LI_CODE];
+    if (!deferred && code == 0 && !S.knobs.test_segflip) pend_clean(S);
     const uint64_t produced = hinfo[LI_OUTLEN];
     if (!direct && produced) INF_CHK(hipMemcpy(out + dict_len, d_out + dict_len, produced, hipMemcpyDeviceToHost));
     *out_len = produced;
@@ -1572,7 +1597,7 @@
     const uint64_t nbits = in_len * 8, nwords = (in_len + 3) / 4;
     const uint32_t* d_w = nullptr;
     INF_RC(stage_input(S, s, in, in_len, flags, &d_w));
-    if (!S.d_stats) INF_CHK(hipMalloc(&S.d_stats, 512));
+    INF_RC(ctl_ensure(S));
     const uint32_t nseg = (uint32_t)std::max<uint64_t>(1, (in_len + SEG_BYTES - 1) / SEG_BYTES);
     INF_CHK(inf_ensure(&S.d_cand, &S.d_cand_cap, (uint64_t)nseg * SEG_CAP * 8ull + (uint64_t)nseg * 4 + 64));
     uint64_t* d_list = (uint64_t*)S.d_cand;
@@ -1628,11 +1653,11 @@
     if (start_bit > nbits) return -1;
     const uint32_t* d_w = nullptr;
     INF_RC(stage_input(S, s, in, in_len, flags, &d_w));
-    if (!S.d_stats) INF_CHK(hipMalloc(&S.d_stats, 512));
+    INF_RC(ctl_ensure(S));
     if (!S.ev[0]) for (auto& e : S.ev) INF_CHK(hipEventCreate(&e));
     int finds = 0;
 refind:
-    INF_CHK(hipMemsetAsync(S.d_stats, 0, 512, s));
+    INF_CHK(hipMemsetAsync(S.d_ctl, 0, CTL_BYTES, s));
     const uint32_t nseg = (uint32_t)std::max<uint64_t>(1, (in_len + SEG_BYTES - 1) / SEG_BYTES);
     INF_CHK(inf_ensure(&S.d_cand, &S.d_cand_cap, (uint64_t)nseg * SEG_CAP * 8ull + (uint64_t)nseg * 4 + 64));
     uint64_t* d_list = (uint64_t*)S.d_cand;
@@ -1721,7 +1746,6 @@
         uint32_t* d_order = (uint32_t*)((char*)S.d_stops + n * 8);
         INF_CHK(hipMemcpyAsync(d_order, order.data(), n * 4, hipMemcpyHostToDevice, s));
         if (!S.d_ph) INF_CHK(hipMalloc(&S.d_ph, (size_t)std::max(COUNT_WAVES, EMIT_WAVES) * sizeof(wv::PhArr)));
-        if (!S.d_cticket) INF_CHK(hipMalloc(&S.d_cticket, CTK_BYTES));
         INF_CHK(hipMemsetAsync(S.d_cticket, 0, 4, s));
         if (S.count_first) INF_CHK(hipEventRecord(S.ev[2], s));
         launch_count(s, count_w(S.knobs), (uint32_t)n,
@@ -1872,8 +1896,7 @@
     if ((nbytes + 31) / 32 > 0xFFFFFFFFull) return -2;
     const uint64_t npw = (nbytes + 31) / 32;
     INF_CHK(inf_ensure(&S.d_ref, &S.d_ref_cap, nbytes * 4 + 64));
-    INF_CHK(inf_ensure(&S.d_pend, &S.d_pend_cap, npw * 4 + 64));
-    INF_CHK(hipMemsetAsync(S.d_pend, 0, npw * 4 + 64, s));
+    INF_RC(pend_prepare(S, s, npw));
     if (!S.h_cnt) INF_CHK(hipHostMalloc(&S.h_cnt, 64, 0));
     hipEvent_t e2 = S.ev[4], e3 = S.ev[5];
     INF_CHK(hipEventRecord(e2, s));
@@ -1936,6 +1959,7 @@
             return (int)er[k].reason;
         }
     }
+    if (!deferred) pend_clean(S);
     if (!direct && total) INF_CHK(hipMemcpy(out + dict_len, d_out + dict_len, total, hipMemcpyDeviceToHost));
     *out_len = total;
     *consumed_bits = stop_bit;
diff --git a/deflate-library-java_amd/csrc/hip/inflate_wave.hpp b/deflate-library-java_amd/csrc/hip/inflate_wave.hpp
--- a/deflate-library-java_amd/csrc/hip/inflate_wave.hpp
+++ b/deflate-library-java_amd/csrc/hip/inflate_wave.hpp
@@ -1321,16 +1321,20 @@
 
 }
 
+#ifndef NDFL_HDR_LANES
+#define NDFL_HDR_LANES 32
+#endif
+static_assert(NDFL_HDR_LANES >= 1 && NDFL_HDR_LANES <= 64, "one wave");
 extern "C" __global__ void __launch_bounds__(64)
 ndfl_inflate_hdr_kernel(const uint32_t* w, uint64_t nwords, uint64_t nbits, const uint64_t* cands, uint32_t ncand,
                         wv::HdrRec* rec, uint32_t* flat_list, uint32_t* nflat, uint32_t* flat_flag) {
     using namespace wv;
-    __shared__ __attribute__((aligned(16))) uint32_t lens[64][80];
-    __shared__ uint16_t clt[64][128];
+    __shared__ __attribute__((aligned(16))) uint32_t lens[NDFL_HDR_LANES][80];
+    __shared__ uint16_t clt[NDFL_HDR_LANES][128];
     __shared__ uint32_t win[8 * 64];
     const uint32_t lane = threadIdx.x;
-    const uint32_t k = blockIdx.x * 64 + lane;
-    if (k >= ncand) return;
+    const uint32_t k = blockIdx.x * NDFL_HDR_LANES + lane;
+    if (lane >= NDFL_HDR_LANES || k >= ncand) return;
     const In in{w, nwords, nbits};
     for (uint32_t q = 0; q < 80; q++) lens[lane][q] = 0;
     const uint64_t p = cands[k];
@@ -2403,8 +2407,9 @@
 
 extern "C" __global__ void __launch_bounds__(256)
 ndfl_inflate_resolve_apply_kernel(const uint32_t* list, const uint32_t* nlist, uint32_t* pend, const uint32_t* newbits,
-                                  uint32_t* list_out, uint32_t* nlist_out, uint32_t* nbytes_out) {
+                                  uint32_t* list_out, uint32_t* nlist_out, uint32_t* nbytes_out, uint32_t* zero_next) {
     const uint32_t n = *nlist;
+    if (zero_next && blockIdx.x == 0 && threadIdx.x == 0) *zero_next = 0;
     for (uint32_t k0 = blockIdx.x * 256; k0 < n; k0 += gridDim.x * 256) {
         const uint32_t k = k0 + threadIdx.x;
         const bool live = k < n;
@@ -2419,7 +2424,10 @@
 }
 
 extern "C" __global__ void __launch_bounds__(256)
-ndfl_inflate_pending_list_kernel(const uint32_t* pend, uint64_t w0, uint64_t w1, uint32_t* list, uint32_t* nlist) {
+ndfl_inflate_pending_list_kernel(const uint32_t* pend, uint64_t w0, uint64_t w1, uint32_t* list, uint32_t* nlist,
+                                 const uint64_t* total, uint64_t dict_len) {
+    if (total) w1 = min(w1, (dict_len + *total + 31) >> 5);
+    if (w0 + (uint64_t)blockIdx.x * 4096 >= w1) return;
     __shared__ uint32_t sh[4], sbase;
     const uint64_t base = w0 + ((uint64_t)blockIdx.x * 256 + threadIdx.x) * 16;
     uint32_t v[16];
```

Measured after the change: 230,100 (median of 6 runs). Within noise of the previous version (+0.7%).
